# lucidrains/flash-cosine-sim-attention

Measured on AMD Instinct MI355X. Metric: attention TFLOP/s fwd+bwd (B=4,H=8,N=4096,D=64 bf16) + max-|delta| vs PyTorch ref, higher is better.
Workload: dtype bf16

## Files before the change

flash_cosine_sim_attention_amd/_lib.py:

```python
from __future__ import annotations

import ctypes as C
import os
import subprocess
import sys

_HERE = os.path.dirname(os.path.abspath(__file__))
LIB_PATH = os.environ.get("FCSA_LIB") or os.path.join(_HERE, "libfcsa_hip.so")
CSRC = os.path.join(_HERE, "csrc")

FCSA_F32, FCSA_F16, FCSA_BF16 = 0, 1, 2
_HEADER_CANDIDATES = (os.path.join(_HERE, "include", "fcsa.h"), os.path.join(os.path.dirname(_HERE), "include", "fcsa.h"))
HEADER = next((h for h in _HEADER_CANDIDATES if os.path.isfile(h)), _HEADER_CANDIDATES[0])



_SCALARS = {"int32_t": C.c_int32, "int64_t": C.c_int64, "uint64_t": C.c_uint64, "float": C.c_float, "size_t": C.c_size_t,
            "char": C.c_char, "int": C.c_int}


def _parse_header(path):
    import re
    text = re.sub(r"/\*.*?\*/", "", open(path).read(), flags=re.S)
    macros = {m.group(1): int(m.group(2)) for m in re.finditer(r"#define\s+(FCSA_\w+)\s+(-?\d+)\s*$", text, flags=re.M)}
    structs = {}
    for m in re.finditer(r"typedef\s+struct\s+(\w+)\s*\{(.*?)\}\s*(\w+)\s*;", text, flags=re.S):
        fields = []
        for decl in m.group(2).split(";"):
            decl = " ".join(decl.split())
            if not decl:
                continue
            head, _, names = decl.rpartition(" ")
            while "," in head:
                head, _, more = head.rpartition(" ")
                names = more + " " + names
            base = head.replace("const", "").strip()
            for nm in names.replace(",", " ").split():
                stars = base.count("*") + nm.count("*")
                nm = nm.strip("*")
                tname = base.replace("*", "").strip()
                arr = re.match(r"(\w+)\[(\d+)\]$", nm)
                if stars:
                    ct = C.c_void_p
                elif tname in structs:
                    ct = structs[tname][1]
                else:
                    ct = _SCALARS[tname]
                if arr:
                    nm, ct = arr.group(1), ct * int(arr.group(2))
                fields.append((nm, ct))
        cls = type(m.group(3), (C.Structure,), {"_fields_": fields})
        structs[m.group(3)] = (fields, cls)
    return {k: v[1] for k, v in structs.items()}, macros


_STRUCTS, _MACROS = _parse_header(HEADER)
ABI_VERSION = _MACROS["FCSA_ABI_VERSION"]
Tensor = _STRUCTS["fcsa_tensor"]
Problem = _STRUCTS["fcsa_problem"]
NormState = _STRUCTS["fcsa_norm_state"]
ForwardArgs = _STRUCTS["fcsa_forward_args"]
BackwardArgs = _STRUCTS["fcsa_backward_args"]
KernelStat = _STRUCTS["fcsa_kernel_stat"]
Varlen = _STRUCTS["fcsa_varlen"]
KvCache = _STRUCTS["fcsa_kvcache"]
Window = _STRUCTS["fcsa_window"]
KvCacheQuant = _STRUCTS["fcsa_kvcache_quant"]
FCSA_CACHE_E4M3 = _MACROS["FCSA_CACHE_E4M3"]
LseOut = _STRUCTS["fcsa_lse_out"]
MergeArgs = _STRUCTS["fcsa_merge_args"]
MERGE_MAX_STATES = _MACROS["FCSA_MERGE_MAX_STATES"]
MergeBackwardArgs = _STRUCTS["fcsa_merge_backward_args"]
KvCacheStep = _STRUCTS["fcsa_kvcache_step"]
STEP_CHUNK_ROWS = _MACROS["FCSA_STEP_CHUNK_ROWS"]
TreeMask = _STRUCTS["fcsa_tree_mask"]
Alibi = _STRUCTS["fcsa_alibi"]


EXPORTS = ("fcsa_forward", "fcsa_backward", "fcsa_backward_workspace_bytes", "fcsa_forward_workspace_bytes", "fcsa_forward_needs_qn",
           "fcsa_l2norm", "fcsa_debug", "fcsa_debug_forward_form", "fcsa_debug_kv_group_form", "fcsa_last_error", "fcsa_profile_enable", "fcsa_profile_collect",
           "fcsa_forward_varlen", "fcsa_backward_varlen", "fcsa_backward_varlen_workspace_bytes", "fcsa_forward_kvcache",
           "fcsa_forward_kvcache_workspace_bytes", "fcsa_forward_window", "fcsa_backward_window", "fcsa_backward_window_workspace_bytes",
           "fcsa_forward_kvcache_window", "fcsa_forward_kvcache_window_workspace_bytes", "fcsa_forward_kvcache_quant",
           "fcsa_forward_kvcache_quant_workspace_bytes", "fcsa_forward_kvcache_varlen", "fcsa_forward_kvcache_varlen_workspace_bytes",
           "fcsa_forward_kvcache_lse", "fcsa_merge_states", "fcsa_forward_kvcache_prefill",
           "fcsa_attention_lse", "fcsa_backward_state", "fcsa_merge_states_backward",
           "fcsa_forward_kvcache_step", "fcsa_forward_kvcache_step_workspace_bytes",
           "fcsa_forward_kvcache_tree", "fcsa_kvcache_compact", "fcsa_forward_kvcache_alibi")

_lib = None


def build(verbose: bool = False) -> str:
    cmd = ["make", "-C", CSRC, "-j", str(min(8, os.cpu_count() or 1)), "PYTHON=" + sys.executable]
    res = subprocess.run(cmd, capture_output=True, text=True)
    if verbose or res.returncode != 0:
        print(res.stdout)
        print(res.stderr)
    if res.returncode != 0:
        raise RuntimeError("building libfcsa_hip.so failed (see output above)")
    return LIB_PATH


def load():
    global _lib
    if _lib is not None:
        return _lib
    if not os.path.exists(LIB_PATH):
        raise ImportError(
            f"{LIB_PATH} is missing: the HIP extension has not been built. Run `make -C {CSRC}` "
            "(or `python -c 'import __graft_entry__ as g; g.build()'` at the repo root). "
            "There is no non-HIP fallback for GPU tensors.")
    lib = C.CDLL(LIB_PATH)
    lib.fcsa_forward.argtypes = [C.POINTER(ForwardArgs)]
    lib.fcsa_forward.restype = C.c_int
    lib.fcsa_backward.argtypes = [C.POINTER(BackwardArgs)]
    lib.fcsa_backward.restype = C.c_int
    lib.fcsa_backward_workspace_bytes.argtypes = [C.POINTER(Problem)]
    lib.fcsa_backward_workspace_bytes.restype = C.c_size_t
    lib.fcsa_forward_workspace_bytes.argtypes = [C.POINTER(Problem)]
    lib.fcsa_forward_workspace_bytes.restype = C.c_size_t
    lib.fcsa_forward_needs_qn.argtypes = [C.POINTER(Problem), C.c_int32]
    lib.fcsa_forward_needs_qn.restype = C.c_int
    lib.fcsa_l2norm.argtypes = [C.c_int32, C.c_int32, C.c_int32, C.c_int32, C.c_int32, C.c_int32,
                                C.POINTER(Tensor), C.c_void_p, C.c_void_p, C.c_void_p]
    lib.fcsa_l2norm.restype = C.c_int
    lib.fcsa_debug.argtypes = [C.c_char_p, C.c_size_t]
    lib.fcsa_debug.restype = C.c_int
    lib.fcsa_debug_forward_form.argtypes = [C.c_int32]
    lib.fcsa_debug_forward_form.restype = C.c_int
    lib.fcsa_debug_kv_group_form.argtypes = [C.c_int32]
    lib.fcsa_debug_kv_group_form.restype = C.c_int
    lib.fcsa_profile_enable.argtypes = [C.c_int32]
    lib.fcsa_profile_enable.restype = C.c_int
    lib.fcsa_profile_collect.argtypes = [C.POINTER(KernelStat), C.c_int32]
    lib.fcsa_profile_collect.restype = C.c_int
    lib.fcsa_forward_varlen.argtypes = [C.POINTER(ForwardArgs), C.POINTER(Varlen)]
    lib.fcsa_forward_varlen.restype = C.c_int
    lib.fcsa_backward_varlen.argtypes = [C.POINTER(BackwardArgs), C.POINTER(Varlen)]
    lib.fcsa_backward_varlen.restype = C.c_int
    lib.fcsa_backward_varlen_workspace_bytes.argtypes = [C.POINTER(Problem), C.POINTER(Varlen)]
    lib.fcsa_backward_varlen_workspace_bytes.restype = C.c_size_t
    lib.fcsa_forward_kvcache.argtypes = [C.POINTER(ForwardArgs), C.POINTER(KvCache)]
    lib.fcsa_forward_kvcache.restype = C.c_int
    lib.fcsa_forward_kvcache_workspace_bytes.argtypes = [C.POINTER(Problem), C.POINTER(KvCache)]
    lib.fcsa_forward_kvcache_workspace_bytes.restype = C.c_size_t
    if hasattr(lib, "fcsa_forward_window"):
        lib.fcsa_forward_window.argtypes = [C.POINTER(ForwardArgs), C.POINTER(Varlen), C.POINTER(Window)]
        lib.fcsa_forward_window.restype = C.c_int
        lib.fcsa_backward_window.argtypes = [C.POINTER(BackwardArgs), C.POINTER(Varlen), C.POINTER(Window)]
        lib.fcsa_backward_window.restype = C.c_int
        lib.fcsa_backward_window_workspace_bytes.argtypes = [C.POINTER(Problem), C.POINTER(Varlen), C.POINTER(Window)]
        lib.fcsa_backward_window_workspace_bytes.restype = C.c_size_t
        lib.fcsa_forward_kvcache_window.argtypes = [C.POINTER(ForwardArgs), C.POINTER(KvCache), C.POINTER(Window)]
        lib.fcsa_forward_kvcache_window.restype = C.c_int
        lib.fcsa_forward_kvcache_window_workspace_bytes.argtypes = [C.POINTER(Problem), C.POINTER(KvCache), C.POINTER(Window)]
        lib.fcsa_forward_kvcache_window_workspace_bytes.restype = C.c_size_t
    if hasattr(lib, "fcsa_forward_kvcache_quant"):
        lib.fcsa_forward_kvcache_quant.argtypes = [C.POINTER(ForwardArgs), C.POINTER(KvCache), C.POINTER(KvCacheQuant), C.POINTER(Window)]
        lib.fcsa_forward_kvcache_quant.restype = C.c_int
        lib.fcsa_forward_kvcache_quant_workspace_bytes.argtypes = [C.POINTER(Problem), C.POINTER(KvCache), C.POINTER(KvCacheQuant),
                                                                   C.POINTER(Window)]
        lib.fcsa_forward_kvcache_quant_workspace_bytes.restype = C.c_size_t
    if hasattr(lib, "fcsa_forward_kvcache_varlen"):
        lib.fcsa_forward_kvcache_varlen.argtypes = [C.POINTER(ForwardArgs), C.POINTER(KvCache), C.POINTER(Varlen), C.POINTER(KvCacheQuant),
                                                    C.POINTER(Window)]
        lib.fcsa_forward_kvcache_varlen.restype = C.c_int
        lib.fcsa_forward_kvcache_varlen_workspace_bytes.argtypes = [C.POINTER(Problem), C.POINTER(KvCache), C.POINTER(Varlen),
                                                                    C.POINTER(KvCacheQuant), C.POINTER(Window)]
        lib.fcsa_forward_kvcache_varlen_workspace_bytes.restype = C.c_size_t
    if hasattr(lib, "fcsa_forward_kvcache_lse"):
        lib.fcsa_forward_kvcache_lse.argtypes = [C.POINTER(ForwardArgs), C.POINTER(KvCache), C.POINTER(Varlen), C.POINTER(KvCacheQuant),
                                                 C.POINTER(Window), C.POINTER(LseOut)]
        lib.fcsa_forward_kvcache_lse.restype = C.c_int
        lib.fcsa_merge_states.argtypes = [C.POINTER(MergeArgs)]
        lib.fcsa_merge_states.restype = C.c_int
    if hasattr(lib, "fcsa_forward_kvcache_prefill"):
        lib.fcsa_forward_kvcache_prefill.argtypes = [C.POINTER(ForwardArgs), C.POINTER(KvCache), C.POINTER(Varlen), C.POINTER(LseOut)]
        lib.fcsa_forward_kvcache_prefill.restype = C.c_int
    if hasattr(lib, "fcsa_attention_lse"):
        lib.fcsa_attention_lse.argtypes = [C.POINTER(Problem), C.c_void_p, C.POINTER(Varlen), C.POINTER(Window), C.POINTER(LseOut), C.c_void_p]
        lib.fcsa_attention_lse.restype = C.c_int
        lib.fcsa_backward_state.argtypes = [C.POINTER(BackwardArgs), C.POINTER(Varlen), C.POINTER(Window), C.c_void_p]
        lib.fcsa_backward_state.restype = C.c_int
        lib.fcsa_merge_states_backward.argtypes = [C.POINTER(MergeBackwardArgs)]
        lib.fcsa_merge_states_backward.restype = C.c_int
    if hasattr(lib, "fcsa_forward_kvcache_step"):
        lib.fcsa_forward_kvcache_step.argtypes = [C.POINTER(ForwardArgs), C.POINTER(KvCache), C.POINTER(Varlen), C.POINTER(KvCacheQuant),
                                                  C.POINTER(Window), C.POINTER(KvCacheStep), C.POINTER(LseOut)]
        lib.fcsa_forward_kvcache_step.restype = C.c_int
        lib.fcsa_forward_kvcache_step_workspace_bytes.argtypes = [C.POINTER(Problem), C.POINTER(KvCache), C.POINTER(Varlen),
                                                                  C.POINTER(KvCacheQuant), C.POINTER(Window), C.POINTER(KvCacheStep)]
        lib.fcsa_forward_kvcache_step_workspace_bytes.restype = C.c_size_t
    if hasattr(lib, "fcsa_forward_kvcache_alibi"):
        lib.fcsa_forward_kvcache_alibi.argtypes = [C.POINTER(ForwardArgs), C.POINTER(KvCache), C.POINTER(Varlen), C.POINTER(KvCacheQuant),
                                                   C.POINTER(Window), C.POINTER(KvCacheStep), C.POINTER(Alibi), C.POINTER(LseOut)]
        lib.fcsa_forward_kvcache_alibi.restype = C.c_int
    if hasattr(lib, "fcsa_forward_kvcache_tree"):
        lib.fcsa_forward_kvcache_tree.argtypes = [C.POINTER(ForwardArgs), C.POINTER(KvCache), C.POINTER(Varlen), C.POINTER(KvCacheQuant),
                                                  C.POINTER(TreeMask), C.POINTER(LseOut)]
        lib.fcsa_forward_kvcache_tree.restype = C.c_int
        lib.fcsa_kvcache_compact.argtypes = [C.POINTER(KvCache), C.c_int32, C.c_int32, C.c_int32, C.c_int32, C.c_void_p, C.c_int64, C.c_int32,
                                             C.c_void_p, C.c_void_p]
        lib.fcsa_kvcache_compact.restype = C.c_int
    lib.fcsa_last_error.argtypes = []
    lib.fcsa_last_error.restype = C.c_char_p
    ver = lib.fcsa_debug(None, 0)
    if ver != ABI_VERSION:
        raise ImportError(f"libfcsa_hip.so ABI version {ver} != expected {ABI_VERSION}; rebuild it")
    _lib = lib
    return lib


def check(rc: int, what: str):
    if rc != 0:
        msg = load().fcsa_last_error().decode("utf-8", "replace")
        raise RuntimeError(f"{what} failed (status {rc}): {msg}")


def forward_form(form: int) -> int:
    return int(load().fcsa_debug_forward_form(int(form)))


def kv_group_form(form: int) -> int:
    return int(load().fcsa_debug_kv_group_form(int(form)))


def source_sha256() -> str:
    import hashlib
    h = hashlib.sha256()
    names = [f for f in sorted(os.listdir(CSRC)) if f.endswith((".hip", ".cuh", ".h", ".cpp")) or f == "Makefile"]
    names += ["dev/" + f for f in sorted(os.listdir(os.path.join(CSRC, "dev")))]
    for name, path in [(n, os.path.join(CSRC, n)) for n in names] + [(os.path.basename(HEADER), HEADER)]:
        h.update(name.encode() + b"\0")
        h.update(open(path, "rb").read())
    return h.hexdigest()


def profile_enable(on: bool):
    check(load().fcsa_profile_enable(1 if on else 0), "fcsa_profile_enable")


def profile_collect():
    arr = (KernelStat * 16)()
    n = load().fcsa_profile_collect(arr, 16)
    if n < 0:
        raise RuntimeError("fcsa_profile_collect failed")
    return [dict(name=arr[i].name.decode(), calls=arr[i].calls, total_ms=arr[i].total_ms, min_ms=arr[i].min_ms,
                 max_ms=arr[i].max_ms) for i in range(min(n, 16))]



def dtype_code(torch_dtype) -> int:
    import torch
    return {torch.float32: FCSA_F32, torch.float16: FCSA_F16, torch.bfloat16: FCSA_BF16}[torch_dtype]


def tensor4(t) -> "Tensor":
    assert t.dim() == 4 and t.stride(3) == 1
    return Tensor(t.data_ptr(), t.stride(0), t.stride(1), t.stride(2))


def problem(torch_dtype, dims, causal=False, bias_batch=False, l2norm_qk=True, groups=1, scale=8.0) -> "Problem":
    B, H, Hk, N, M, D = dims
    return Problem(dtype_code(torch_dtype), B, H, Hk, N, M, D, int(bool(causal)), int(bool(bias_batch)),
                   int(bool(l2norm_qk)), int(groups if l2norm_qk else 1), float(scale))


def forward_needs_qn(prob: "Problem", need_backward: bool) -> bool:
    return bool(load().fcsa_forward_needs_qn(C.byref(prob), 1 if need_backward else 0))
```

flash_cosine_sim_attention_amd/csrc/fcsa_bwd.hip:

```cpp
#include <type_traits>

#include "fcsa_common.cuh"
#include "fcsa_kernels.h"

namespace fcsa {
constexpr int kDqSub8 = 4;
constexpr bool kDqSplitFirstStage = true;
constexpr int kDkvBmq8 = 128;
constexpr int kDkvBmqWide = 64;
constexpr bool kDkvRing = true;
FCSA_TRACE_SITE(dq)
FCSA_TRACE_SITE(dkv)

template <typename T, int D, int MODE, bool BIAS, bool TWO, bool WIN = false>
FCSA_DEV void dq_tile(const char* kt, const char* vt, const FragAddr<T, D>& fa,
                      const u32x4 (&qf)[TileGeom<D, Traits<T>::ES>::KS], const u32x4 (&dof)[TileGeom<D, Traits<T>::ES>::KS],
                      f32x16 (&dq)[TileGeom<D, Traits<T>::ES>::DB], float lc, float delta, const BwdParams& p, uint64_t word,
                      uint32_t ncm, int i, int j0, int diff, const char* bias_row, int m_lim, int dlo = 0) {
  typedef TileGeom<D, Traits<T>::ES> G;
  typedef Traits<T> TR;
  constexpr bool MASKED = MODE == 1, KEYM = MODE == 2;
#pragma unroll
  for (int jb = 0; jb < 2; ++jb) {
    uint32_t w = 0xffffffffu;
// ... 1155 lines not shown
        reinterpret_cast<float*>(buf + 2 * TILE_B + BMQ * 4)[tid] = row_ok ? -dl_r : 0.f;
      }
    }
  };

  if constexpr (!DMA) {
    if (t0 < QT) load_tile(t0, smem);
  }

  u32x4 kf[G::KS], vf[G::KS];
#pragma unroll
  for (int kk = 0; kk < G::KS; ++kk) {
    kf[kk] = p.q_scaled ? rk_[kk] : scale_frag<T>(rk_[kk], p.c1);
    if constexpr (!LEAN) vf[kk] = rv_[kk];
  }
  float rinv[RowEpilogue<T, D>::NP];
  if constexpr (SEP) {
#pragma unroll
    for (int e = 0; e < RowEpilogue<T, D>::NP; ++e) rinv[e] = rinv_n[e];
  }
  const bool key_ok = j < p.M && rmask != 0;
  const uint32_t kmask = key_ok ? 0xffffffffu : 0u;
  const uint32_t ncm = causal ? 0u : 0xffffffffu;

  f32x16 dk[G::DB], dv[G::DB];
#pragma unroll
  for (int db = 0; db < G::DB; ++db)
#pragma unroll
    for (int r = 0; r < 16; ++r) { dk[db][r] = 0.f; dv[db][r] = 0.f; }

  if (t0 < QT) store_tile(smem);
  if constexpr (RING) {
    if ((SWEEP ? t0 < QT && (t0 + 1 < QT || p.kv_group > 1) : t0 + 1 < QT) && tid < BMQ) {
      char* buf1 = smem + BUF_B;
      reinterpret_cast<float*>(buf1 + 2 * TILE_B)[tid] = row_ok2 ? (p.invl_log2 ? lc_r2 : __builtin_amdgcn_logf(lc_r2)) - p.c2 : -INFINITY;
      reinterpret_cast<float*>(buf1 + 2 * TILE_B + BMQ * 4)[tid] = row_ok2 ? -dl_r2 : 0.f;
    }
  }
  if constexpr (LEAN) dma_wait();
  __syncthreads();
  __builtin_amdgcn_s_waitcnt(0x0F70);

  int t_m = QT;
  if (!BIAS && p.mask == nullptr && n0 + BNK <= p.M) {
    t_m = t0;
    if (causal) t_m = min(QT, max(t0, (nw + 31 - diff - hq + BMQ - 1) / BMQ));
  }
  int t_e = QT;
  if constexpr (WIN) win_unmasked_query_tiles(t0, QT, n0 + BNK <= p.M, nw, hq, BMS, BMQ, diff, dlo, t_m, t_e);
  const bool head_skip0 = SWEEP && causal && t_m > t0 && t0 * BMQ + hq + BMS - 1 + diff < nw;

  tr.loop_begin();
  DkvPipe<T, D, BMS> pipe;
  int pipe_tile = -1;
  int ring = 0;
  int tpar = 0;
  int gi = 0;
  auto run = [&](auto masked_tag, int t_begin, int t_end) {
    constexpr int MODE = decltype(masked_tag)::value;
    constexpr bool MASKED = MODE != 0;
    for (int t = t_begin; t < t_end; ++t) {
      const int i0 = t * BMQ;
      const int par = RING ? ring : SWEEP ? tpar : (t - t0) & 1;
      const int par_nxt = RING ? (ring == 2 ? 0 : ring + 1) : (par ^ 1);
      const int par_ld = RING ? (ring == 0 ? 2 : ring - 1) : (par ^ 1);
      const int t_ld = RING ? t + 2 : t + 1;
      const char* cur = smem + par * BUF_B;
      char* nxt = smem + par_ld * BUF_B;
      bool more = t_ld < QT;
      FCSA_STAMP(ts, 0);
      const float* lcs = reinterpret_cast<const float*>(cur + 2 * TILE_B);
      const float* dls = lcs + BMQ;
      if constexpr (SWEEP) {
        more = cursor_next(t0);
        if (more) load_rows(lt * BMQ);
      } else if constexpr (DMA) {
        if (more) {
          advance(t_ld);
          load_rows(t_ld * BMQ);
        }
      }
      if constexpr (DMA) {
        const uint32_t lds_nxt = lds0 + par_ld * BUF_B;
        FCSA_STAMP(ts, 1);
        if (more) {
          dq_.issue(stq, lds_nxt, wave);
          ddo_.issue(stdo, lds_nxt + TILE_B, wave);
        }
      } else {
        if (more) load_tile(t + 1, nxt);
        FCSA_STAMP(ts, 1);
      }
      {
      bool skip = false;
      if constexpr (MASKED) skip = causal && (i0 + hq + BMS - 1 + diff < nw);
      if constexpr (MASKED && WIN) skip = skip || (i0 + hq > nw + 31 - dlo);
      if constexpr (PIPE) {
        if constexpr (RING) {
          if (!skip) {
            const bool has_next = t + 1 < QT || (SWEEP && gi + 1 < p.kv_group && !head_skip0);
            if constexpr (QSPLIT)
              dkv_tile_pipe<T, D, BMS, tile_mode<MODE>(), true, true, WIN>(cur + hoff, cur + TILE_B + hoff, lcs + hq, dls + hq, fa, kf, vf, dk, dv, kmask, ncm, j, i0 + hq, diff, ts,
                                                          pipe, pipe_tile != t, has_next ? smem + par_nxt * BUF_B : cur, wave >= 4, hoff, hq, dlo);
            else
            dkv_tile_pipe<T, D, BMQ, tile_mode<MODE>(), true, false, WIN>(cur, cur + TILE_B, lcs, dls, fa, kf, vf, dk, dv, kmask, ncm, j, i0, diff, ts, pipe, pipe_tile != t,
                                                  has_next ? smem + par_nxt * BUF_B : cur, NW == 8 && wave >= 4, 0, 0, dlo);
            pipe_tile = has_next ? (t + 1 < QT ? t + 1 : t0) : -1;
          }
          ring = par_nxt;
        } else {
          if (!skip) dkv_tile_pipe<T, D, BMQ, tile_mode<MODE>(), false, false, WIN>(cur, cur + TILE_B, lcs, dls, fa, kf, vf, dk, dv, kmask, ncm, j, i0, diff, ts, pipe, true, nullptr,
                                                    NW == 8 && wave >= 4, 0, 0, dlo);
        }
      } else if constexpr (LEAN) {
        if (!skip) dkv_tile<T, D, BMQ, tile_mode<MODE>(), false, true, WIN>(cur, cur + TILE_B, lcs, dls, fa, kf, vf, dk, dv, p, kmask, ncm, j, i0, diff, nullptr, ts,
                                                            bb, bscr, nullptr, false, -1, lane, smem + LDS::VOWN, wave * 32, NW == 8 && wave >= 4, dlo);
      } else {
        const int next_i0 = more ? i0 + hq + BMQ : -1;
        if (!skip) {
          dkv_tile<T, D, BMS, tile_mode<MODE>(), BIAS, false, WIN>(cur + hoff, cur + TILE_B + hoff, lcs + hq, dls + hq, fa, kf, vf, dk, dv, p, kmask, ncm, j, i0 + hq, diff, bias_col, ts, bb, bscr,
                                            bias_blk, bvec, next_i0, lane, nullptr, 0, false, dlo);
        } else if constexpr (BIAS) {
          if (bvec && more) bb.request(bias_blk, min(next_i0 + (lane & 31), p.N - 1), (int64_t)p.M * TR::ES, fa.hi);
        }
      }
      }
      FCSA_STAMP(ts, 8);
      if (more) store_tile(nxt);
      if constexpr (SWEEP) tpar ^= 1;
      FCSA_STAMP(ts, 9);
      FCSA_BAR_BEGIN(tr);
      __syncthreads();
      FCSA_BAR_END(tr);
      FCSA_STAMP(ts, 10);
      if constexpr (!MASKED) ts.close(10);
    }
  };
  tr.mark(pass, 1);
  tpar = 0;
  for (gi = 0; gi < (SWEEP ? p.kv_group : 1); ++gi) {
    if constexpr (WIN) {
      int sb = t0, se = t_m, ub = t_m, ue = t_e;
#pragma nounroll
      for (int seg = 0; seg < 2; ++seg) {
        run(std::integral_constant<int, 1>{}, sb, se);
        run(std::integral_constant<int, 0>{}, ub, ue);
        sb = t_e; se = QT; ub = QT; ue = QT;
      }
    } else {
    run(std::integral_constant<int, KM ? 2 : 1>{}, t0, t_m);
    tr.mark(pass, 2);
    run(std::integral_constant<int, 0>{}, t_m, QT);
    }
  }
  tr.mark(pass, 3);
  tr.loop_end();

  if constexpr (QSPLIT) {
    LDS::HO::run(smem, rwave, half, lane, [&](int n) { return acc_x4(n & 4 ? dv : dk, n / 8 * 4 + n % 4); },
                 [&](int n, const f32x4& v) { add_x4(n & 4 ? dv : dk, n / 8 * 4 + n % 4, v); });
  }
  {
    typedef RowEpilogue<T, D> EP;
    char* scr = LDS::scratch(smem, rwave);
    char* xs = LDS::xarea(smem, rwave);
    const int rows_valid = half == 0 ? p.M - nw : 0;
    const bool fused = p.rk != nullptr;
    const int le = opaque(lane);
    const float kmul = p.q_scaled ? p.scale / p.c1 : p.scale;
    if constexpr (!SEP) {
#pragma unroll
      for (int e = 0; e < EP::NP; ++e) rinv[e] = 1.f;
      if (fused && rows_valid > 0) EP::load_inv(rinv, p.rk + (rk_bh * p.M + nw) * p.G, p.G, p.lgm, le, rows_valid);
    }
    if (rows_valid > 0) EP::put(scr, dk, kmul, le, (LDS::X && fused) ? kf : nullptr, xs, LDS::XPITCH);
    have_pre = false;
    if constexpr (SEP) {
      if (pass + 1 < npass) {
        request_ahead(pass + 1);
        have_pre = true;
      }
    }
    if (rows_valid > 0) {
      const int64_t split_off = p.dkv_splits > 1 ? (int64_t)blockIdx.y * p.dkv_split_stride : 0;
      const int ho = SWEEP ? hk : h;
      char* dk0 = p.dk.p + (int64_t)b * p.dk.sb + (int64_t)ho * p.dk.sh + (int64_t)nw * p.dk.sn + split_off;
      char* dv0 = p.dv.p + (int64_t)b * p.dv.sb + (int64_t)ho * p.dv.sh + (int64_t)nw * p.dv.sn + split_off;
      const char* x0 = fused ? p.k.p + (int64_t)b * p.k.sb + (int64_t)hk * p.k.sh + (int64_t)nw * p.k.sn : nullptr;
      EP::template finish<LDS::X>(scr, xs, LDS::XPITCH, le, dk0, p.dk.sn, rows_valid, fused ? false : p.dk_f32 != 0, x0, p.k.sn, 1.f, rinv, p.lgm,
                                  p.norm_eps);
      EP::put(scr, dv, 1.f, le, nullptr, xs, LDS::XPITCH);
      EP::template finish<false>(scr, xs, LDS::XPITCH, le, dv0, p.dv.sn, rows_valid, p.dv_f32 != 0, nullptr, 0, 1.f, rinv, 0, 1.f);
    }
    if constexpr (!SEP) {
      if (pass + 1 < npass) __syncthreads();
    }
  }
  tr.mark(pass, 4);
  }
  tr.finish(ts, wave, (wave & 2) == 0, trace_row8(wave));
}

template <typename T, int D, int NW, int BMQ, bool BIAS, bool LEAN, bool KM, bool RING = false, bool QSPLIT = false, bool SWEEP = false>
__global__ void __launch_bounds__(NW * 64, ((D * Traits<T>::ES <= kDkv2WBytes || LEAN) ? 2 : 1)) bwd_dkv_kernel(const BwdParams p_) {
  bwd_dkv_body<T, D, NW, BMQ, BIAS, LEAN, KM, RING, QSPLIT, SWEEP, false>(p_);
}
template <typename T, int D, int NW, int BMQ, bool LEAN, bool RING, bool QSPLIT>
__global__ void __launch_bounds__(NW * 64, ((D * Traits<T>::ES <= kDkv2WBytes || LEAN) ? 2 : 1)) bwd_dkv_win_kernel(const BwdWinParams p_) {
  bwd_dkv_body<T, D, NW, BMQ, false, LEAN, false, RING, QSPLIT, false, true>(p_);
}

template <typename T, int D, bool BIAS, int NW, bool TWO, bool KSPLIT = false>
static hipError_t launch_dq_nw(const BwdWinParams& p, hipStream_t s) {
  constexpr int SUB = KSPLIT ? 2 : NW == 8 ? (Traits<T>::ES == 2 ? kDqSub8 : 2) : 1;
  typedef DqLds<T, D, NW, SUB, TWO, KSPLIT> LDS;
  const dim3 grid((unsigned)((int64_t)p.B * p.H * tile_pairs(tile_count(p.N, 32 * LDS::RWAVES), p.causal)), (unsigned)(p.dq_splits > 1 ? p.dq_splits : 1));
  constexpr bool GENERAL_ONLY = TWO && D * Traits<T>::ES >= 256;
  if (p.window) {
    if constexpr (!BIAS && !(TWO && D * Traits<T>::ES > kDq2WBytes)) {
      if (!p.causal || p.dq_splits > 1 || p.mask != nullptr) return hipErrorInvalidValue;
      return launch_with_lds<bwd_dq_win_kernel<T, D, NW, SUB, TWO, KSPLIT>>(grid, dim3(NW * 64), LDS::TOTAL, s, p);
    }
    return hipErrorInvalidValue;
  }
  const BwdParams& bp = p;
  if constexpr (!GENERAL_ONLY) {
    if (!p.causal) return launch_with_lds<bwd_dq_kernel<T, D, NW, BIAS, SUB, TWO, true, KSPLIT>>(grid, dim3(NW * 64), LDS::TOTAL, s, bp);
  }
  return launch_with_lds<bwd_dq_kernel<T, D, NW, BIAS, SUB, TWO, false, KSPLIT>>(grid, dim3(NW * 64), LDS::TOTAL, s, bp);
}

template <typename T, int D, bool BIAS>
static hipError_t launch_dq_form(DqForm f, const BwdWinParams& p, hipStream_t s) {
  constexpr int ES = Traits<T>::ES;
  constexpr bool NARROW = D * ES <= kDq2WBytes;
  switch (f) {
    case DqForm::Waves4:
      return launch_dq_nw<T, D, BIAS, 4, NARROW>(p, s);
    case DqForm::Waves4Two:
      if constexpr (NARROW || (dq_can_two_waves(ES, D) && !BIAS)) return launch_dq_nw<T, D, BIAS, 4, true>(p, s);
      break;
    case DqForm::Waves8:
      if constexpr (NARROW) return launch_dq_nw<T, D, BIAS, 8, true>(p, s);
      break;
    case DqForm::KSplit8:
      if constexpr (bwd_ksplit(ES, D, false) && (NARROW || (dq_can_two_waves(ES, D) && !BIAS))) return launch_dq_nw<T, D, BIAS, 8, true, true>(p, s);
      break;
  }
  return hipErrorInvalidValue;
}

template <typename T, int D, bool BIAS, int NW, bool LEAN = false, bool QSPLIT = false, bool SWEEP = false>
static hipError_t launch_dkv_nw(const BwdWinParams& p, hipStream_t s) {
  constexpr bool DMA_FORM = Traits<T>::ES == 2 && !BIAS;
  constexpr int LEAN_BMQ = D * Traits<T>::ES < 256 ? 64 : 32;
  constexpr int BMQ = LEAN ? LEAN_BMQ : (D * Traits<T>::ES >= 192) ? (DMA_FORM ? kDkvBmqWide : 32) : (NW == 8 ? kDkvBmq8 : 64);
  constexpr bool RING = kDkvRing && DMA_FORM && !LEAN && (BMQ * TileGeom<D, Traits<T>::ES>::ROWB) % 1024 == 0 &&
                        DkvLds<T, D, NW, BMQ, BIAS, false, true, false>::FITS;
  typedef DkvLds<T, D, NW, BMQ, BIAS, LEAN, RING, QSPLIT> LDS;
  const dim3 grid((unsigned)(p.B * (SWEEP ? p.H / p.kv_group : p.H) * tile_pairs(tile_count(p.M, 32 * LDS::RWAVES), p.causal)),
                  (unsigned)(p.dkv_splits > 1 ? p.dkv_splits : 1));
  if (p.window) {
    if constexpr (!BIAS && !SWEEP) {
      if (!p.causal || p.dkv_splits > 1 || p.mask != nullptr) return hipErrorInvalidValue;
      return launch_with_lds<bwd_dkv_win_kernel<T, D, NW, BMQ, LEAN, RING, QSPLIT>>(grid, dim3(NW * 64), LDS::TOTAL, s, p);
    }
    return hipErrorInvalidValue;
  }
  const BwdParams& bp = p;
  return p.causal ? launch_with_lds<bwd_dkv_kernel<T, D, NW, BMQ, BIAS, LEAN, false, RING, QSPLIT, SWEEP>>(grid, dim3(NW * 64), LDS::TOTAL, s, bp)
                  : launch_with_lds<bwd_dkv_kernel<T, D, NW, BMQ, BIAS, LEAN, true, RING, QSPLIT, SWEEP>>(grid, dim3(NW * 64), LDS::TOTAL, s, bp);
}

static std::atomic<int> g_kv_group_mode{1};
int kv_group_mode(int set) {
  if (set < 0) return g_kv_group_mode.load(std::memory_order_relaxed);
  return g_kv_group_mode.exchange(set > 2 ? 2 : set, std::memory_order_relaxed);
}

template <typename T, int D, bool BIAS>
static hipError_t launch_dkv_form(DkvForm f, const BwdWinParams& p, hipStream_t s) {
  constexpr int ES = Traits<T>::ES;
  constexpr bool NARROW = D * ES <= kDkv2WBytes;
  switch (f) {
    case DkvForm::Waves4:
      return launch_dkv_nw<T, D, BIAS, 4>(p, s);
    case DkvForm::Waves8:
      if constexpr (NARROW) return launch_dkv_nw<T, D, BIAS, 8>(p, s);
      break;
    case DkvForm::Lean8:
      if constexpr (ES == 2 && !BIAS && !NARROW && D * ES <= 256) return launch_dkv_nw<T, D, BIAS, 8, true>(p, s);
      break;
    case DkvForm::QSplit8:
      if constexpr (NARROW && bwd_ksplit(ES, D, false)) return launch_dkv_nw<T, D, BIAS, 8, false, true>(p, s);
      break;
    case DkvForm::Sweep:
      if constexpr (dkv_has_sweep(ES, D, BIAS)) return launch_dkv_nw<T, D, BIAS, 8, !NARROW, false, true>(p, s);
      break;
  }
  return hipErrorInvalidValue;
}

static BwdProblem bwd_problem(int dtype, int D, const BwdWinParams& p, int splits) {
  return {dtype == 0 ? 4 : 2, D, (int64_t)p.B * p.H, p.N, p.M, p.causal != 0, p.bias != nullptr, splits, p.kv_sweep != 0,
          p.seq.cu_q != nullptr || p.window != 0, p.window != 0};
}

hipError_t launch_backward_dbias(int dtype, int D, const BwdParams& p, hipStream_t s) {
  if (p.B * p.H == 0 || p.N == 0 || p.M == 0 || p.d_bias == nullptr || p.bias == nullptr) return hipSuccess;
  return dispatch_dtype_d(dtype, D, [&](auto td) { return launch_dbias_t<typename decltype(td)::T, decltype(td)::D>(p, s); });
}

hipError_t launch_backward_dq(int dtype, int D, const BwdWinParams& p, hipStream_t s) {
  if (p.B * p.H == 0 || p.N == 0) return hipSuccess;
  const DqForm f = choose_dq(bwd_problem(dtype, D, p, p.dq_splits), cu_count());
  return dispatch_dtype_d(dtype, D, [&](auto td) {
    using T = typename decltype(td)::T;
    constexpr int DD = decltype(td)::D;
    return p.bias != nullptr ? launch_dq_form<T, DD, true>(f, p, s) : launch_dq_form<T, DD, false>(f, p, s);
  });
}

hipError_t launch_backward_dkv(int dtype, int D, const BwdWinParams& p, hipStream_t s) {
  if (p.B * p.H == 0 || p.M == 0) return hipSuccess;
  const DkvForm f = choose_dkv(bwd_problem(dtype, D, p, p.dkv_splits), cu_count());
  return dispatch_dtype_d(dtype, D, [&](auto td) {
    using T = typename decltype(td)::T;
    constexpr int DD = decltype(td)::D;
    return p.bias != nullptr ? launch_dkv_form<T, DD, true>(f, p, s) : launch_dkv_form<T, DD, false>(f, p, s);
  });
}

}
```

flash_cosine_sim_attention_amd/csrc/fcsa_capi.hip:

```cpp
#include "../../include/fcsa.h"
#include "fcsa_kernels.h"

#include <algorithm>
#include <cstdarg>
#include <cstdio>
#include <cmath>
#include <cstring>
#include <atomic>
#include <mutex>
#include <string>
#include <vector>

namespace {

thread_local std::string g_err;
constexpr float kLog2e = 1.4426950408889634f;

int fail(int code, const char* fmt, ...) {
  char buf[512];
  va_list ap;
  va_start(ap, fmt);
  vsnprintf(buf, sizeof(buf), fmt, ap);
  va_end(ap);
  g_err = buf;
  return code;
}

int elem_size(int dtype) { return dtype == FCSA_F32 ? 4 : 2; }

size_t align_up(size_t x, size_t a) { return (x + a - 1) / a * a; }

bool dim_ok(int d) { return d == 16 || d == 32 || d == 64 || d == 96 || d == 128; }

int check_problem(const fcsa_problem& p) {
  if (p.dtype != FCSA_F16 && p.dtype != FCSA_BF16 && p.dtype != FCSA_F32)
    return fail(FCSA_ERR_UNSUPPORTED, "unsupported dtype %d (expected f32=0, f16=1, bf16=2)", p.dtype);
  if (!dim_ok(p.dim_head))
    return fail(FCSA_ERR_UNSUPPORTED, "dim_head %d not in {16, 32, 64, 96, 128}", p.dim_head);
  if (p.batch < 0 || p.heads < 0 || p.q_len < 0 || p.k_len < 0)
    return fail(FCSA_ERR_INVALID_ARG, "negative size (B=%d H=%d N=%d M=%d)", p.batch, p.heads, p.q_len, p.k_len);
  if (p.kv_heads < 1 ? p.heads != 0 || p.kv_heads != 0 : p.heads % p.kv_heads != 0)
    return fail(FCSA_ERR_INVALID_ARG, "kv_heads must divide heads (%d), got %d", p.heads, p.kv_heads);
  if (p.l2norm_qk) {
    if (p.groups < 1 || p.dim_head % p.groups != 0)
      return fail(FCSA_ERR_INVALID_ARG, "groups (%d) must divide dim_head (%d)", p.groups, p.dim_head);
    if (p.dtype == FCSA_F16 && fabsf(p.scale) * kLog2e > 60000.f)
      return fail(FCSA_ERR_UNSUPPORTED, "float16: scale %g puts scale * log2(e) * q^ outside the type", (double)p.scale);
  } else if (p.groups != 1) {
    return fail(FCSA_ERR_INVALID_ARG, "groups must be 1 when l2norm_qk is 0");
  }
  if (!(p.scale == p.scale) || std::isinf(p.scale)) return fail(FCSA_ERR_INVALID_ARG, "scale is NaN or infinite");
  return FCSA_OK;
}

int check_tensor(const char* name, const fcsa_tensor& t, int es, bool required) {
  if (t.ptr == nullptr) return required ? fail(FCSA_ERR_INVALID_ARG, "%s: null pointer", name) : FCSA_OK;
  if ((reinterpret_cast<uintptr_t>(t.ptr) & 15) != 0) return fail(FCSA_ERR_INVALID_ARG, "%s: base not 16-byte aligned", name);
  const int64_t m = 16 / es;
  if (t.stride0 % m || t.stride1 % m || t.stride2 % m)
    return fail(FCSA_ERR_INVALID_ARG, "%s: strides (%lld, %lld, %lld) must keep rows 16-byte aligned", name,
                (long long)t.stride0, (long long)t.stride1, (long long)t.stride2);
  if (t.stride2 < 0 || t.stride2 * es > (int64_t)(0x3fffffff / 256))
    return fail(FCSA_ERR_UNSUPPORTED, "%s: row stride %lld elements is negative or above 4 MiB", name, (long long)t.stride2);
  return FCSA_OK;
}

fcsa::View view(const fcsa_tensor& t, int es, bool zero_head_stride = false) {
  fcsa::View v;
  v.p = static_cast<char*>(t.ptr);
  v.sb = t.stride0 * es;
  v.sh = zero_head_stride ? 0 : t.stride1 * es;
  v.sn = t.stride2 * es;
  return v;
}

fcsa::View contiguous_view(void* p, int64_t heads, int64_t len, int64_t d, int es, bool zero_head_stride = false) {
  fcsa::View v;
  v.p = static_cast<char*>(p);
  v.sb = heads * len * d * es;
  v.sh = zero_head_stride ? 0 : len * d * es;
  v.sn = d * es;
  return v;
}

constexpr float kStaticTop = 65.f, kStaticBottom = 85.f;
constexpr float kStaticBoundBias = 40.f;
bool dynamic_shift(const fcsa_problem& p, bool has_bias) {
  if (!p.l2norm_qk) return false;
  const float bound = fabsf(p.scale) * (float)p.groups;
  if (p.dtype == FCSA_F16) return has_bias || bound > 11.f;
  return 2.f * bound > kStaticTop + kStaticBottom || (has_bias && bound > kStaticBoundBias);
}

float exponent_shift(const fcsa_problem& p, bool has_bias) {
  if (!p.l2norm_qk) return p.scale;
  if (dynamic_shift(p, has_bias)) return 0.f;
  const float bound = fabsf(p.scale) * (float)p.groups;
  if (p.dtype == FCSA_F16) return bound - 10.f;
  const float lo = bound - kStaticTop, hi = kStaticBottom - bound;
  return p.scale < lo ? lo : (p.scale > hi ? hi : p.scale);
}

float rowsum_eps(const fcsa_problem& p, bool has_bias) {
  if (dynamic_shift(p, has_bias)) return 1e-30f;
  float e = 1e-10f * expf(p.scale - exponent_shift(p, has_bias));
  if (!(e > 1e-37f)) e = 1e-37f;
  if (e > 1e30f) e = 1e30f;
  return e;
}

int log2_blocks_per_group(const fcsa_problem& p) {
  const int dg = p.dim_head / (p.groups > 0 ? p.groups : 1);
  if (dg % 8 != 0) return -1;
  int m = dg / 8, lg = 0;
  while ((1 << lg) < m) ++lg;
  if (p.groups <= 1) return lg;
  return (1 << lg) == m ? lg : -1;
}
bool fusable_groups(const fcsa_problem& p) { return log2_blocks_per_group(p) >= 0; }

struct BwdPlan {
  bool fuse_norm;
  bool kv_sweep;
  int dq_splits;
  int dkv_splits;
  bool dq_slab, dk_slab, dv_slab;
};
struct BwdCall { bool bias, dq_flat, dkv_flat; };

BwdPlan bwd_plan(const fcsa_problem& p, const BwdCall* call, bool varlen = false) {
  BwdPlan b;
  const int cus = fcsa::cu_count();
  const bool grouped = p.kv_heads != p.heads;
  const bool sweep = !varlen && p.kv_heads > 1 && grouped && (p.l2norm_qk == 0 || fusable_groups(p)) &&
                     fcsa::dkv_sweep(elem_size(p.dtype), p.dim_head, (int64_t)p.batch * p.kv_heads, p.k_len, p.causal != 0, fcsa::kv_group_mode(-1), cus);
  b.kv_sweep = sweep && call != nullptr && !call->bias;
  b.fuse_norm = p.l2norm_qk != 0 && fusable_groups(p);
  const bool norm_slab = p.l2norm_qk != 0 && !b.fuse_norm;
  b.dq_splits = varlen || (call != nullptr && !(call->dq_flat && !(p.causal && call->bias))) ? 1 : fcsa::backward_dq_splits(p, cus);
  b.dkv_splits = varlen || sweep || (call != nullptr && !((call->dkv_flat || grouped) && !call->bias)) ? 1 : fcsa::backward_dkv_splits(p, cus);
  b.dq_slab = b.dq_splits > 1 || norm_slab;
  b.dk_slab = !b.kv_sweep && (b.dkv_splits > 1 || grouped || norm_slab);
  b.dv_slab = !b.kv_sweep && (b.dkv_splits > 1 || grouped);
  return b;
}

struct BwdLayout { size_t delta, dq_slab, dk_slab, dv_slab, total; };
BwdLayout bwd_layout(const fcsa_problem& p, bool varlen = false) {
  const BwdPlan b = bwd_plan(p, nullptr, varlen);
  const size_t qn = (size_t)p.batch * p.heads * p.q_len;
  const size_t kn = (size_t)p.batch * p.heads * p.k_len;
  BwdLayout L;
  size_t off = 0;
  L.delta = off;   off = align_up(off + qn * 4, 256);
  L.dq_slab = off; off = align_up(off + (b.dq_slab ? qn * p.dim_head * 4 * (size_t)b.dq_splits : 0), 256);
  L.dk_slab = off; off = align_up(off + (b.dk_slab ? kn * p.dim_head * 4 * (size_t)b.dkv_splits : 0), 256);
  L.dv_slab = off; off = align_up(off + (b.dv_slab ? kn * p.dim_head * 4 * (size_t)b.dkv_splits : 0), 256);
  L.total = off;
  return L;
}

int launch_check(hipError_t e, const char* what) {
  if (e != hipSuccess) return fail(FCSA_ERR_LAUNCH, "%s: %s", what, hipGetErrorString(e));
  return FCSA_OK;
}

struct TimedLaunch { const char* name; hipEvent_t start, stop; };
std::mutex g_prof_mu;
std::atomic<bool> g_prof_on{false};
std::vector<TimedLaunch> g_prof;

template <typename F> int timed(const char* name, const char* what, hipStream_t s, F&& launch) {
  if (!g_prof_on.load(std::memory_order_relaxed)) return launch_check(launch(), what);
  TimedLaunch t{name, nullptr, nullptr};
  if (hipEventCreate(&t.start) != hipSuccess || hipEventCreate(&t.stop) != hipSuccess)
    return fail(FCSA_ERR_LAUNCH, "%s: hipEventCreate failed", what);
  (void)hipEventRecord(t.start, s);
  const hipError_t e = launch();
  (void)hipEventRecord(t.stop, s);
  { std::lock_guard<std::mutex> g(g_prof_mu); g_prof.push_back(t); }
  return launch_check(e, what);
}

int check_varlen(const fcsa_problem& p, const fcsa_varlen* v, bool mask, bool bias) {
  if (v == nullptr) return fail(FCSA_ERR_INVALID_ARG, "varlen: null sequence table");
  if (mask || bias) return fail(FCSA_ERR_INVALID_ARG, "varlen: mask and attn_bias are not supported with packed sequences");
  if (v->total_q < 0 || v->total_k < 0 || v->total_q > INT32_MAX || v->total_k > INT32_MAX)
    return fail(FCSA_ERR_INVALID_ARG, "varlen: total_q / total_k (%lld, %lld) outside [0, 2^31)", (long long)v->total_q, (long long)v->total_k);
  if (p.batch > 0 && (v->cu_seqlens_q == nullptr || v->cu_seqlens_k == nullptr))
    return fail(FCSA_ERR_INVALID_ARG, "varlen: null cu_seqlens");
  if ((int64_t)p.heads * (v->total_q > v->total_k ? v->total_q : v->total_k) > INT32_MAX)
    return fail(FCSA_ERR_UNSUPPORTED, "varlen: heads x packed rows above 2^31");
  return FCSA_OK;
}
fcsa_problem packed_problem(const fcsa_problem& p, const fcsa_varlen& v) {
  fcsa_problem d = p;
  d.batch = 1;
  d.q_len = (int32_t)v.total_q;
  d.k_len = (int32_t)v.total_k;
  return d;
}
struct VarlenCall { const fcsa_varlen* t; int batch, max_q, max_k; };
fcsa::SeqTable seq_table(const VarlenCall* v) {
  if (v == nullptr) return fcsa::SeqTable{nullptr, nullptr, 0, 0};
  return fcsa::SeqTable{v->t->cu_seqlens_q, v->t->cu_seqlens_k, (int)v->t->total_q, (int)v->t->total_k};
}
fcsa_tensor packed(fcsa_tensor t) {
  t.stride0 = 0;
  return t;
}

struct WindowCall { int lo, hi; };
int check_window(const fcsa_window* w, bool mask, bool bias) {
  if (w == nullptr) return fail(FCSA_ERR_INVALID_ARG, "window: null window");
  if (w->left < -1 || w->right < -1) return fail(FCSA_ERR_INVALID_ARG, "window: left / right (%d, %d) must be >= 0, or -1 for unbounded", w->left, w->right);
  if (mask || bias) return fail(FCSA_ERR_INVALID_ARG, "window: mask and attn_bias are not supported with a sliding window");
  return FCSA_OK;
}

int forward_impl(const fcsa_forward_args* a, const VarlenCall* vl, const WindowCall* win = nullptr);
int backward_impl(const fcsa_backward_args* a, const VarlenCall* vl, const WindowCall* win = nullptr, const float* dlse = nullptr);

}

extern "C" {

const char* fcsa_last_error(void) { return g_err.c_str(); }

int fcsa_profile_enable(int32_t enable) {
  g_prof_on.store(enable != 0, std::memory_order_relaxed);
  return FCSA_OK;
}

int fcsa_profile_collect(fcsa_kernel_stat* stats, int32_t capacity) {
  std::vector<TimedLaunch> rec;
  { std::lock_guard<std::mutex> g(g_prof_mu); rec.swap(g_prof); }
  std::vector<fcsa_kernel_stat> agg;
  for (TimedLaunch& t : rec) {
    float ms = 0.f;
    const bool ok = hipEventSynchronize(t.stop) == hipSuccess && hipEventElapsedTime(&ms, t.start, t.stop) == hipSuccess;
    (void)hipEventDestroy(t.start);
    (void)hipEventDestroy(t.stop);
    if (!ok) continue;
    fcsa_kernel_stat* st = nullptr;
    for (auto& a : agg) if (strcmp(a.name, t.name) == 0) st = &a;
    if (st == nullptr) {
      fcsa_kernel_stat n;
      memset(&n, 0, sizeof(n));
      strncpy(n.name, t.name, sizeof(n.name) - 1);
      n.min_ms = ms; n.max_ms = ms;
      agg.push_back(n);
      st = &agg.back();
    }
    st->calls += 1;
    st->total_ms += ms;
    if (ms < st->min_ms) st->min_ms = ms;
    if (ms > st->max_ms) st->max_ms = ms;
  }
  if (stats != nullptr)
    for (int i = 0; i < (int)agg.size() && i < capacity; ++i) stats[i] = agg[i];
  return (int)agg.size();
}

int fcsa_debug(char* buf, size_t buf_bytes) {
  if (buf != nullptr && buf_bytes > 0) {
    snprintf(buf, buf_bytes,
             "libfcsa_hip abi=%d arch=gfx950 dtypes=f32,f16,bf16 dim_head=16,32,64,96,128 "
             "kernels=l2norm,l2norm_pair,fwd(32 rows/wave; lean two-wave form at D=96/128),fwd2(64 rows/wave),fwd3(D=128: 64 rows/wave, 1 wave/SIMD),fwd_ksplit(128 rows, wave halves split the keys),fwd_split+combine,"
             "fwd_dyn(per-row shift),bwd_dq(+split-key; key-split form on 8 waves),bwd_dkv(+lean; query-split form on 8 waves; grouped-query K/V head sweep),bwd_dbias,finalize,kv_append+decode+decode_combine(kv cache),"
             "window(fwd_win,bwd_dq_win,bwd_dkv_win,decode_win: sliding-window forms),"
             "kv_append_fp8+decode_fp8+decode_combine_fp8(e4m3fn kv cache, f16/bf16 queries),"
             "kv_append_ragged+decode_ragged+decode_combine_ragged(+_fp8: packed queries with per-sequence counts against the kv cache),"
             "decode_tree(+_fp8: a per-row bit set over the step's tokens, tree attention for speculative decoding)+kv_compact(the accepted path to the front of its slots) kv_heads=divisors of heads",
             FCSA_ABI_VERSION);
  }
  return FCSA_ABI_VERSION;
}

int fcsa_debug_forward_form(int32_t form) { return fcsa::forward_wide128_mode(form); }

int fcsa_debug_kv_group_form(int32_t form) { return fcsa::kv_group_mode(form); }

int fcsa_l2norm(int32_t dtype, int32_t batch, int32_t heads, int32_t len, int32_t dim_head, int32_t groups,
                const fcsa_tensor* x, void* xn, float* inv_norm, void* stream) {
  if (dtype != FCSA_F16 && dtype != FCSA_BF16 && dtype != FCSA_F32) return fail(FCSA_ERR_UNSUPPORTED, "fcsa_l2norm: dtype %d not supported", dtype);
  if (batch < 0 || heads < 0 || len < 0) return fail(FCSA_ERR_INVALID_ARG, "fcsa_l2norm: negative size (B=%d H=%d L=%d)", batch, heads, len);
  if (batch == 0 || heads == 0 || len == 0) return FCSA_OK;
  if (x == nullptr || xn == nullptr) return fail(FCSA_ERR_INVALID_ARG, "fcsa_l2norm: null argument");
  if (dim_head <= 0 || dim_head % 8 != 0) return fail(FCSA_ERR_UNSUPPORTED, "fcsa_l2norm: dim_head %d must be a multiple of 8", dim_head);
  if (dim_head > 512) return fail(FCSA_ERR_UNSUPPORTED, "fcsa_l2norm: dim_head %d > 512", dim_head);
  if (groups < 1 || dim_head % groups != 0) return fail(FCSA_ERR_INVALID_ARG, "fcsa_l2norm: groups (%d) must divide dim_head (%d)", groups, dim_head);
  const int es = elem_size(dtype);
  if (int rc = check_tensor("x", *x, es, true)) return rc;
  fcsa::NormParams np;
  np.x = view(*x, es);
  np.xn = static_cast<char*>(xn);
  np.inv_norm = inv_norm;
  np.B = batch; np.H = heads; np.L = len; np.D = dim_head; np.G = groups;
  np.eps = 1e-12f;
  np.out_scale = 1.f;
  hipStream_t s = static_cast<hipStream_t>(stream);
  return timed("l2norm", "l2norm", s, [&] { return fcsa::launch_l2norm(dtype, np, s); });
}

static int forward_splits(const fcsa_problem& p) {
  if (p.batch <= 0 || p.heads <= 0 || p.q_len <= 0 || p.dim_head <= 0) return 1;
  return fcsa::forward_splits(p, dynamic_shift(p, false), fcsa::cu_count());
}
static size_t forward_ws_bytes(const fcsa_problem& p, int splits) {
  if (splits <= 1) return 0;
  const size_t rows = (size_t)splits * p.batch * p.heads * p.q_len;
  return align_up(rows * p.dim_head * 4, 256) + align_up(rows * 4, 256);
}

size_t fcsa_forward_workspace_bytes(const fcsa_problem* p) { return p == nullptr ? 0 : forward_ws_bytes(*p, forward_splits(*p)); }

static int zero_rows(const char* name, const fcsa_tensor& t, int es, int B, int H, int L, int D, hipStream_t s) {
  if (B <= 0 || H <= 0 || L <= 0) return FCSA_OK;
  if (int rc = check_tensor(name, t, es, true)) return rc;
  for (int b = 0; b < B; ++b)
    for (int h = 0; h < H; ++h) {
      char* base = static_cast<char*>(t.ptr) + ((int64_t)b * t.stride0 + (int64_t)h * t.stride1) * es;
      const hipError_t e = t.stride2 == D ? hipMemsetAsync(base, 0, (size_t)L * D * es, s)
                                          : hipMemset2DAsync(base, (size_t)t.stride2 * es, 0, (size_t)D * es, (size_t)L, s);
      if (e != hipSuccess) return fail(FCSA_ERR_LAUNCH, "%s: zero fill failed: %s", name, hipGetErrorString(e));
    }
  return FCSA_OK;
}

int fcsa_forward(const fcsa_forward_args* a) { return forward_impl(a, nullptr); }

static int forward_varlen(const fcsa_forward_args* a, const fcsa_varlen* seqs, const WindowCall* win) {
  if (a == nullptr) return fail(FCSA_ERR_INVALID_ARG, "null args");
  if (int rc = check_problem(a->p)) return rc;
  if (int rc = check_varlen(a->p, seqs, a->mask != nullptr, a->attn_bias != nullptr)) return rc;
  fcsa_forward_args pa = *a;
  pa.q = packed(pa.q); pa.k = packed(pa.k); pa.v = packed(pa.v); pa.o = packed(pa.o);
  pa.p = packed_problem(a->p, *seqs);
  const VarlenCall vl = {seqs, a->p.batch, a->p.q_len, a->p.k_len};
  return forward_impl(&pa, &vl, win);
}
int fcsa_forward_varlen(const fcsa_forward_args* a, const fcsa_varlen* seqs) { return forward_varlen(a, seqs, nullptr); }

int fcsa_forward_window(const fcsa_forward_args* a, const fcsa_varlen* seqs, const fcsa_window* w) {
  if (a == nullptr) return fail(FCSA_ERR_INVALID_ARG, "null args");
  if (int rc = check_problem(a->p)) return rc;
  if (int rc = check_window(w, a->mask != nullptr, a->attn_bias != nullptr)) return rc;
  WindowCall win;
  const fcsa::WinKind kind = fcsa::win_normalise(a->p.q_len, a->p.k_len, a->p.causal != 0, w->left, w->right, win.lo, win.hi);
  if (kind == fcsa::WinKind::Window) return seqs != nullptr ? forward_varlen(a, seqs, &win) : forward_impl(a, nullptr, &win);
  fcsa_forward_args na = *a;
  na.p.causal = kind == fcsa::WinKind::Causal ? 1 : 0;
  return seqs != nullptr ? fcsa_forward_varlen(&na, seqs) : fcsa_forward(&na);
}


}

namespace {

struct DecodeCall {
  const fcsa_forward_args* a;
  const fcsa_kvcache* kv;
  const fcsa_varlen* seqs;
  const fcsa_kvcache_quant* qz;
  const fcsa_window* w;
  const fcsa_lse_out* lse;
  const fcsa_kvcache_step* step = nullptr;
  const fcsa_tree_mask* tree = nullptr;
  const fcsa_alibi* alibi = nullptr;
};

struct DecodeWindow {
  int windowed, lo, hi, causal;
  int reach() const { return windowed ? lo : fcsa::kWinOpen; }
};
DecodeWindow decode_window(const fcsa_problem& p, const fcsa_kvcache& kv, bool ragged, const fcsa_window* w) {
  if (ragged) {
    const int lo = w == nullptr || w->left < 0 ? fcsa::kWinOpen : std::min(w->left, fcsa::kWinOpen);
    const int hi = p.causal ? 0 : (w == nullptr || w->right < 0 ? fcsa::kWinOpen : std::min(w->right, fcsa::kWinOpen));
    return {1, lo, hi, p.causal};
  }
  if (w == nullptr) return {0, 0, 0, p.causal};
  int lo, hi;
  const int max_k = std::min(std::max(p.k_len, 0), std::max(kv.capacity, 0));
  const fcsa::WinKind kind = fcsa::win_normalise(p.q_len, max_k, p.causal != 0, w->left, w->right, lo, hi);
  if (kind == fcsa::WinKind::Window) return {1, lo, hi, p.causal};
  return {0, 0, 0, kind == fcsa::WinKind::Causal ? 1 : 0};
}

struct DecodePlan { int row_tiles; int64_t slots; int splits; size_t ws_ml, total; };
DecodePlan decode_plan(const fcsa_problem& p, const fcsa_kvcache& kv, const fcsa_varlen* seqs, int win_lo, int64_t decode_rows = -1) {
  DecodePlan d;
  const int G = p.kv_heads > 0 ? p.heads / p.kv_heads : 0;
  const int max_k = fcsa::win_decode_keys(std::min(std::max(p.k_len, 0), std::max(kv.capacity, 0)), std::max(p.q_len, 0), win_lo);
  size_t rows;
  if (seqs != nullptr) {
    const int64_t total_q = std::max<int64_t>(seqs->total_q, 0);
    d.row_tiles = 0;
    d.slots = fcsa::ragged_slots(total_q, std::max(p.batch, 0), G);
    const int64_t split_slots = decode_rows < 0 ? d.slots : fcsa::ragged_slots(std::min(decode_rows, total_q), std::max(p.batch, 0), G);
    d.splits = fcsa::decode_splits(1, p.kv_heads, (int)std::min<int64_t>(split_slots, INT32_MAX), max_k, p.dim_head, fcsa::cu_count());
    rows = (size_t)total_q * std::max(p.heads, 0);
  } else {
    d.row_tiles = std::max(fcsa::decode_row_tiles(G * p.q_len), 1);
    d.slots = 0;
    d.splits = fcsa::decode_splits(p.batch, p.kv_heads, d.row_tiles, max_k, p.dim_head, fcsa::cu_count());
    rows = (size_t)std::max(p.batch, 0) * std::max(p.heads, 0) * std::max(p.q_len, 0);
  }
  d.ws_ml = align_up(rows * d.splits * std::max(p.dim_head, 0) * 4, 256);
  d.total = rows == 0 ? 0 : d.ws_ml + align_up(rows * d.splits * 8, 256);
  return d;
}
size_t decode_workspace_bytes(const fcsa_problem* p, const fcsa_kvcache* kv, const fcsa_varlen* seqs, const fcsa_window* w) {
  if (p == nullptr || kv == nullptr) return 0;
  return decode_plan(*p, *kv, seqs, decode_window(*p, *kv, seqs != nullptr, w).reach()).total;
}

int check_kvcache(const fcsa_forward_args* a, const fcsa_kvcache* kv, int cache_es = 0) {
  if (a == nullptr || kv == nullptr) return fail(FCSA_ERR_INVALID_ARG, "kvcache: null argument");
  const fcsa_problem& p = a->p;
  if (int rc = check_problem(p)) return rc;
  if (a->inv_l != nullptr || a->mask != nullptr || a->attn_bias != nullptr)
    return fail(FCSA_ERR_INVALID_ARG, "kvcache: inv_l, mask and attn_bias must be NULL (forward only, no mask or bias)");
  if (kv->capacity < 0 || kv->new_len < 0) return fail(FCSA_ERR_INVALID_ARG, "kvcache: negative capacity (%d) or new_len (%d)", kv->capacity, kv->new_len);
  if (kv->block_table != nullptr) {
    if (kv->page_size <= 0 || kv->page_size % 16 != 0) return fail(FCSA_ERR_INVALID_ARG, "kvcache: page_size %d must be a positive multiple of 16", kv->page_size);
    if (kv->capacity % kv->page_size != 0) return fail(FCSA_ERR_INVALID_ARG, "kvcache: capacity %d is not a whole number of pages of %d", kv->capacity, kv->page_size);
    if (kv->capacity > 0 && kv->num_blocks < 1) return fail(FCSA_ERR_INVALID_ARG, "kvcache: paged cache without blocks");
    if (kv->block_table_stride < kv->capacity / kv->page_size) return fail(FCSA_ERR_INVALID_ARG, "kvcache: block_table row stride %lld below %d entries", (long long)kv->block_table_stride, kv->capacity / kv->page_size);
  } else if (kv->page_size != 0) {
    return fail(FCSA_ERR_INVALID_ARG, "kvcache: page_size %d without a block_table", kv->page_size);
  }
  const int es = elem_size(p.dtype);
  const bool rows = p.batch > 0 && p.heads > 0 && p.q_len > 0;
  const bool cache = p.batch > 0 && kv->capacity > 0;
  const int ces = cache_es > 0 ? cache_es : es;
  if (rows) {
    if (int rc = check_tensor("q", a->q, es, true)) return rc;
    if (int rc = check_tensor("o", a->o, es, true)) return rc;
  }
  if (cache) {
    if (int rc = check_tensor("k_cache", kv->k_cache, ces, true)) return rc;
    if (int rc = check_tensor("v_cache", kv->v_cache, ces, true)) return rc;
  }
  if (cache && kv->new_len > 0) {
    if (int rc = check_tensor("k_new", kv->k_new, es, true)) return rc;
    if (int rc = check_tensor("v_new", kv->v_new, es, true)) return rc;
  }
  if (rows) {
    const DecodePlan d = decode_plan(p, *kv, nullptr, fcsa::kWinOpen);
    if ((int64_t)p.batch * p.kv_heads * d.row_tiles * d.splits > INT32_MAX) return fail(FCSA_ERR_UNSUPPORTED, "kvcache: grid above 2^31 workgroups");
  }
  return FCSA_OK;
}

int check_quant(const fcsa_forward_args* a, const fcsa_kvcache* kv, const fcsa_kvcache_quant* qz) {
  if (a == nullptr || kv == nullptr || qz == nullptr) return fail(FCSA_ERR_INVALID_ARG, "kvcache_quant: null argument");
  if (qz->cache_dtype != FCSA_CACHE_E4M3)
    return fail(FCSA_ERR_UNSUPPORTED, "kvcache_quant: cache type %d not supported (expected FCSA_CACHE_E4M3 = %d, OCP e4m3fn)", qz->cache_dtype, FCSA_CACHE_E4M3);
  if (a->p.dtype == FCSA_F32) return fail(FCSA_ERR_UNSUPPORTED, "kvcache_quant: float32 queries with an fp8 cache are not supported (f16 or bf16)");
  if (qz->k_scale == nullptr || qz->v_scale == nullptr) return fail(FCSA_ERR_INVALID_ARG, "kvcache_quant: null k_scale / v_scale");
  return check_kvcache(a, kv, 1);
}

int check_kvcache_varlen(const DecodeCall& c) {
  const fcsa_forward_args* a = c.a;
  const fcsa_kvcache* kv = c.kv;
  const fcsa_varlen* seqs = c.seqs;
  if (a == nullptr || kv == nullptr || seqs == nullptr) return fail(FCSA_ERR_INVALID_ARG, "kvcache_varlen: null argument");
  if (seqs->total_q < 0 || seqs->total_q > INT32_MAX) return fail(FCSA_ERR_INVALID_ARG, "kvcache_varlen: total_q (%lld) outside [0, 2^31)", (long long)seqs->total_q);
  if (a->p.batch > 0 && seqs->cu_seqlens_q == nullptr) return fail(FCSA_ERR_INVALID_ARG, "kvcache_varlen: null cu_seqlens_q");
  if (kv->new_len != 0 && kv->new_len != 1) return fail(FCSA_ERR_INVALID_ARG, "kvcache_varlen: new_len (%d) is a flag here: 0 (no append) or 1 (every query row brings its key and value)", kv->new_len);
  if (c.w != nullptr)
    if (int rc = check_window(c.w, false, false)) return rc;
  fcsa_forward_args pa = *a;
  fcsa_kvcache pk = *kv;
  pa.q = packed(pa.q); pa.o = packed(pa.o);
  pk.k_new = packed(pk.k_new); pk.v_new = packed(pk.v_new);
  pa.p.q_len = (int32_t)seqs->total_q;
  pa.p.batch = std::min(a->p.batch, 1);
  pk.new_len = kv->new_len != 0 && seqs->total_q > 0 ? 1 : 0;
  if (a->p.q_len < 0) return fail(FCSA_ERR_INVALID_ARG, "kvcache_varlen: negative max_seqlen_q (%d)", a->p.q_len);
  if ((int64_t)std::max(a->p.heads, 0) * seqs->total_q > INT32_MAX) return fail(FCSA_ERR_UNSUPPORTED, "kvcache_varlen: heads x packed rows above 2^31");
  return c.qz != nullptr ? check_quant(&pa, &pk, c.qz) : check_kvcache(&pa, &pk);
}

struct LaunchName { const char* name; const char* what; };
constexpr LaunchName kAppendName[2][2] = {{{"kv_append", "kv append"}, {"kv_append_fp8", "kv append (fp8)"}},
                                          {{"kv_append_ragged", "kv append (ragged)"}, {"kv_append_ragged_fp8", "kv append (ragged)"}}};
constexpr LaunchName kDecodeName[2][2] = {{{"decode", "decode"}, {"decode_fp8", "decode (fp8)"}},
                                          {{"decode_ragged", "decode (ragged)"}, {"decode_ragged_fp8", "decode (ragged)"}}};
constexpr LaunchName kCombineName[2][2][2] = {
    {{{"decode_combine", "decode combine"}, {"decode_combine_lse", "decode combine (lse)"}},
     {{"decode_combine_fp8", "decode combine (fp8)"}, {"decode_combine_lse_fp8", "decode combine (lse, fp8)"}}},
    {{{"decode_combine_ragged", "decode combine (ragged)"}, {"decode_combine_lse_ragged", "decode combine (lse, ragged)"}},
     {{"decode_combine_ragged_fp8", "decode combine (ragged)"}, {"decode_combine_lse_ragged_fp8", "decode combine (lse, ragged)"}}}};

fcsa::DecodeStepParams decode_params(const DecodeCall& c, const DecodeWindow& win, const DecodePlan& d) {
  const bool ragged = c.seqs != nullptr, fp8 = c.qz != nullptr;
  const fcsa_forward_args* a = c.a;
  const fcsa_kvcache* kv = c.kv;
  const fcsa_problem& p = a->p;
  const int es = elem_size(p.dtype), ces = fp8 ? 1 : es;
  auto rows_view = [&](const fcsa_tensor& t) { return view(ragged ? packed(t) : t, es); };
  fcsa::DecodeStepParams dp{};
  dp.q = rows_view(a->q);
  dp.o = rows_view(a->o);
  dp.kc = view(kv->k_cache, ces);
  dp.vc = view(kv->v_cache, ces);
  dp.kn = rows_view(kv->k_new);
  dp.vn = rows_view(kv->v_new);
  dp.seqlens = kv->cache_seqlens;
  dp.table = kv->block_table;
  dp.table_stride = kv->block_table_stride;
  dp.capacity = kv->capacity;
  dp.page = kv->block_table != nullptr ? kv->page_size : 0;
  dp.num_blocks = kv->num_blocks;
  dp.new_len = ragged ? 0 : kv->new_len;
  dp.B = p.batch; dp.H = p.heads; dp.Hk = p.kv_heads; dp.G = p.heads / p.kv_heads; dp.N = ragged ? 0 : p.q_len;
  dp.row_tiles = d.row_tiles; dp.splits = d.splits;
  dp.causal = win.causal; dp.l2norm = p.l2norm_qk; dp.groups = p.l2norm_qk ? p.groups : 1;
  dp.c1 = p.scale * kLog2e;
  dp.c2 = exponent_shift(p, false) * kLog2e;
  dp.l_eps = rowsum_eps(p, false);
  dp.dyn = dynamic_shift(p, false) ? 1 : 0;
  dp.ws_o = static_cast<float*>(a->workspace);
  dp.ws_ml = a->workspace != nullptr ? reinterpret_cast<float*>(static_cast<char*>(a->workspace) + d.ws_ml) : nullptr;
  dp.window = win.windowed; dp.win_lo = win.lo; dp.win_hi = win.hi;
  if (fp8) {
    dp.k_scale = c.qz->k_scale; dp.v_scale = c.qz->v_scale;
    dp.ks_b = c.qz->k_scale_stride0; dp.ks_h = c.qz->k_scale_stride1;
    dp.vs_b = c.qz->v_scale_stride0; dp.vs_h = c.qz->v_scale_stride1;
  }
  if (ragged) {
    dp.cu_q = c.seqs->cu_seqlens_q;
    dp.total_q = (int)c.seqs->total_q;
    dp.slots = (int)d.slots;
    dp.append = kv->new_len != 0 ? 1 : 0;
  }
  if (c.alibi != nullptr) {
    dp.c2 = 0.f;
    dp.l_eps = 1e-30f;
    dp.dyn = 1;
  }
  return dp;
}

fcsa::DecodeLseOut lse_view(const fcsa_lse_out& l, bool packed = false) { return {l.lse, packed ? 0 : l.stride0, l.stride1, l.stride2}; }

bool has_chunk_kernel(const fcsa_problem& p) { return p.dtype != FCSA_F32 && (p.dim_head == 64 || p.dim_head == 128); }

int check_workspace(const char* who, const fcsa_forward_args& a, const DecodePlan& d) {
  if (a.workspace == nullptr || a.workspace_bytes < d.total)
    return fail(FCSA_ERR_WORKSPACE, "%s: workspace too small: %zu < %zu bytes", who, a.workspace_bytes, d.total);
  if ((reinterpret_cast<uintptr_t>(a.workspace) & 255) != 0) return fail(FCSA_ERR_WORKSPACE, "%s: workspace not 256-byte aligned", who);
  return FCSA_OK;
}

int append_launch(const DecodeCall& c, fcsa::DecodeForm form, const fcsa::DecodeStepParams& dp, hipStream_t s) {
  if (c.kv->new_len <= 0 || c.kv->capacity <= 0) return FCSA_OK;
  const LaunchName& n = kAppendName[form.ragged][form.fp8];
  return timed(n.name, n.what, s, [&] { return fcsa::launch_kv_append(c.a->p.dtype, c.a->p.dim_head, form, dp, s); });
}

fcsa::DecodeAlibi alibi_view(const fcsa_alibi& al) { return {al.slopes, al.stride_b, al.stride_h}; }
constexpr LaunchName kAlibiDecodeName[2] = {{"alibi_decode", "decode (alibi)"}, {"alibi_decode_fp8", "decode (alibi, fp8)"}};
constexpr LaunchName kAlibiPrefillName[2] = {{"alibi_prefill", "prefill (alibi)"}, {"alibi_prefill_fp8", "prefill (alibi, fp8)"}};

int decode_launch(const LaunchName& plain, const DecodeCall& c, fcsa::DecodeForm form, const fcsa::DecodeStepParams& dp, hipStream_t s) {
  const fcsa_problem& p = c.a->p;
  if (c.alibi == nullptr) return timed(plain.name, plain.what, s, [&] { return fcsa::launch_decode(p.dtype, p.dim_head, form, dp, s); });
  const LaunchName& n = kAlibiDecodeName[form.fp8];
  const fcsa::DecodeAlibi al = alibi_view(*c.alibi);
  return timed(n.name, n.what, s, [&] { return fcsa::launch_decode_alibi(p.dtype, p.dim_head, form, dp, al, s); });
}

int chunk_launch(const LaunchName& plain, const DecodeCall& c, fcsa::DecodeForm form, fcsa::DecodeStepParams dp, int64_t slots, hipStream_t s) {
  dp.slots = (int)slots;
  dp.splits = 1;
  dp.ws_o = nullptr;
  dp.ws_ml = nullptr;
  const fcsa::DecodeLseOut lo = c.lse != nullptr ? lse_view(*c.lse, true) : fcsa::DecodeLseOut{};
  const fcsa::DecodeLseOut* lse = c.lse != nullptr ? &lo : nullptr;
// ... 684 lines not shown
```

flash_cosine_sim_attention_amd/csrc/fcsa_dispatch.h:

```cpp
#pragma once
#include <stdint.h>
#include <algorithm>
#include <cmath>

#include "../../include/fcsa.h"
#ifdef FCSA_VAR_SPLIT_ENV
#include "dev/fcsa_sweep_env.h"
namespace fcsa {
inline int sweep_env(const char* name) { return fcsa_dev::env_int(name); }
constexpr bool kSweepBuild = true;
}
#else
namespace fcsa {
constexpr int sweep_env(const char*) { return -1; }
constexpr bool kSweepBuild = false;
}
#endif

namespace fcsa {

constexpr int kDq2WBytes = 128;
constexpr int kDkv2WBytes = 128;

constexpr bool fwd_lean(int es, int D, bool bias) { return es == 2 && !bias && D * es > 128 && D * es <= 256; }
// ... 5 lines not shown

enum class FwdForm { Rows8, Lean8, KSplit8, Waves4, Fwd2, Fwd3 };
enum class DqForm { Waves4, Waves4Two, Waves8, KSplit8 };
enum class DkvForm { Waves4, Waves8, Lean8, QSplit8, Sweep };

constexpr int tile_count(int len, int tile) { return (len + tile - 1) / tile; }
constexpr int tile_pairs(int tiles, int causal) { return causal ? (tiles + 1) / 2 : tiles; }
constexpr int pair_passes(int tiles, int pair, int causal) { return (causal && (tiles - 1 - pair) != pair) ? 2 : 1; }
constexpr int pass_tile(int tiles, int pair, int pass, int causal, bool rows) {
  return causal ? (rows ? (pass == 0 ? tiles - 1 - pair : pair) : (pass == 0 ? pair : tiles - 1 - pair)) : pair;
}

constexpr void block_work(int id, int n_bh, int pairs, int& bh, int& pair) {
  if ((n_bh & 7) == 0) {
    const int xcd = id & 7, slot = id >> 3;
    bh = (slot / pairs) * 8 + xcd;
    pair = slot % pairs;
  } else {
    bh = id / pairs;
    pair = id % pairs;
  }
}

constexpr void key_split(int M, int split, int splits, int bn, int& lo, int& len) {
  const int tps = ((M + bn - 1) / bn + splits - 1) / splits;
  lo = split * tps * bn;
  len = std::max(std::min(lo + tps * bn, M) - lo, 0);
}
constexpr void key_split_causal(int N, int M, int m0, int bm, int split, int splits, int bn, int& lo, int& len) {
  const int vis = std::max(std::min(m0 + bm + M - N, M), 0);
  const int tps = std::max(((vis + bn - 1) / bn + splits - 1) / splits, 1);
  lo = std::min(M, split * tps * bn);
  len = std::max(std::min(lo + tps * bn, M) - lo, 0);
}
constexpr int key_tiles(int len, int m0, int bm, int diff, int causal, int bn) {
  int last_key = len - 1;
  if (causal) last_key = std::min(m0 + bm - 1 + diff, last_key);
  return last_key < 0 ? 0 : last_key / bn + 1;
}
constexpr void query_split(int tiles, int split, int splits, int& lo, int& hi) {
  const int tps = (tiles + splits - 1) / splits;
  lo = split * tps;
  hi = std::min(lo + tps, tiles);
}
constexpr int diagonal_tile(int n0, int diff, int bmq) { return std::max(n0 - diff, 0) / bmq; }
constexpr void query_split_causal(int tiles, int first, int split, int splits, int& lo, int& hi) {
  const int tps = std::max((tiles - first + splits - 1) / splits, 1);
  lo = std::min(first + split * tps, tiles);
  hi = std::min(lo + tps, tiles);
}

constexpr int kWinOpen = 1 << 28;
enum class WinKind { Full, Causal, Window };
constexpr WinKind win_normalise(int N, int M, bool causal, int left, int right, int& lo, int& hi) {
  hi = causal ? 0 : (right < 0 || right >= N - 1) ? kWinOpen : right;
  lo = (left < 0 || left >= M - 1) ? kWinOpen : left;
  return lo != kWinOpen ? WinKind::Window : hi == kWinOpen ? WinKind::Full : hi == 0 ? WinKind::Causal : WinKind::Window;
}
constexpr void win_key_window(int N, int M, int m0, int bm, int lo, int hi, int bn, int& k_lo, int& len) {
  const int d = M - N, r1 = std::min(m0 + bm, N) - 1;
  const int first = std::max(m0 + d - lo, 0), last = std::min(r1 + d + hi, M - 1);
  k_lo = 0;
  len = 0;
  if (r1 < m0 || last < first) return;
  k_lo = first / bn * bn;
  len = last + 1 - k_lo;
}
constexpr void win_unmasked_tiles(int len, int nt, int mw, int rows, int diff, int dlo, int bn, int& a, int& b) {
  const int hi_t = std::min(len / bn, std::max(0, mw + diff + 1) / bn);
  const int edge = mw + rows - 1 + dlo;
  a = std::min(edge <= 0 ? 0 : (edge + bn - 1) / bn, nt);
  b = std::max(a, std::min(hi_t, nt));
}
constexpr void win_query_tiles(int N, int M, int n0, int bnk, int lo, int hi, int bmq, int& t0, int& t1) {
  const int d = M - N, k1 = std::min(n0 + bnk, M) - 1;
  const int first = std::max(n0 - d - hi, 0), last = std::min(k1 - d + lo, N - 1);
  t0 = 0;
  t1 = 0;
  if (k1 < n0 || last < first) return;
  t0 = first / bmq;
  t1 = last / bmq + 1;
}
constexpr void win_unmasked_query_tiles(int t0, int t1, bool whole, int nw, int hq, int bms, int bmq, int diff, int dlo, int& a, int& b) {
  a = t1;
  b = t1;
  if (!whole) return;
  a = std::min(t1, std::max(t0, (nw + 31 - diff - hq + bmq - 1) / bmq));
  const int64_t x = (int64_t)nw - dlo - hq - bms + 1;
  b = std::min<int64_t>(t1, std::max<int64_t>(a, x < 0 ? 0 : x / bmq + 1));
}
constexpr void seq_span(int64_t lo, int64_t hi, int total, int max_len, int& start, int& len) {
  const int64_t st = std::min(std::max(lo, (int64_t)0), (int64_t)total);
  const int64_t en = std::min(std::max(hi, st), (int64_t)total);
  start = (int)st;
  len = (int)std::min(en - st, (int64_t)std::max(max_len, 0));
}
constexpr bool seq_pair_idle(int pair, int len, int tile, int causal) { return pair >= tile_pairs(tile_count(len, tile), causal); }

constexpr int kDecodeRows = 16;
constexpr int kDecodeBlock = 32;
constexpr int kDecodeMaxSplits = 128;
constexpr int kDecodeWavesPerCu = 8;
constexpr int decode_row_tiles(int groups_x_queries) { return (groups_x_queries + kDecodeRows - 1) / kDecodeRows; }
constexpr int decode_min_split_keys(int D) { return std::max(16384 / std::max(D, 1), kDecodeBlock); }
inline int decode_splits(int64_t batch, int kv_heads, int row_tiles, int max_k, int D, int cus) {
  const int64_t base = batch * (int64_t)kv_heads * row_tiles;
  if (base <= 0 || max_k <= 0) return 1;
  int64_t s = ((int64_t)cus * kDecodeWavesPerCu + base - 1) / base;
  s = std::min<int64_t>(s, std::max(1, max_k / decode_min_split_keys(D)));
  s = std::min<int64_t>(s, kDecodeMaxSplits);
  return (int)std::max<int64_t>(s, 1);
}
constexpr void decode_window(int len, int split, int splits, int& lo, int& n) {
  const int per = (std::max(len, 0) + splits - 1) / std::max(splits, 1);
  const int chunk = (per + kDecodeBlock - 1) / kDecodeBlock * kDecodeBlock;
  lo = std::min(split * chunk, std::max(len, 0));
  n = std::max(std::min(lo + chunk, len) - lo, 0);
}
constexpr int decode_len(bool has_table, int64_t cached, int new_len, int capacity) {
  const int64_t c = has_table ? std::min<int64_t>(std::max<int64_t>(cached, 0), capacity) : capacity;
  return (int)std::min<int64_t>(c + std::max(new_len, 0), capacity);
}
constexpr bool decode_groups_fast(int D, int groups, int unit) {
  if (groups < 1 || D % groups != 0) return false;
  const int gs = D / groups;
  if (groups == 1 || unit % gs == 0) return true;
  if (gs % unit != 0) return false;
  const int u = gs / unit;
  return (u & (u - 1)) == 0;
}

constexpr int win_decode_first(int len, int N, int lo) {
  return lo >= kWinOpen ? 0 : std::max(len - N - lo, 0) / kDecodeBlock * kDecodeBlock;
}
constexpr int win_decode_keys(int max_k, int N, int lo) {
  return lo >= kWinOpen ? max_k : (int)std::min<int64_t>(max_k, (int64_t)lo + N + kDecodeBlock - 1);
}

constexpr int64_t ragged_cu(int64_t raw, int64_t total) { return std::min(std::max(raw, (int64_t)0), total); }
constexpr int64_t ragged_base(int64_t cu_b, int b, int G) { return (int64_t)G * cu_b / kDecodeRows + b; }
constexpr int64_t ragged_slots(int64_t total_q, int64_t B, int G) { return (int64_t)G * total_q / kDecodeRows + B; }
constexpr int ragged_seq_of(const int32_t* cu, int B, int64_t total, int64_t tok) {
  int lo = 0, hi = B - 1;
  while (lo < hi) {
    const int mid = (lo + hi + 1) / 2;
    if (ragged_cu(cu[mid], total) <= tok) lo = mid; else hi = mid - 1;
  }
  return lo;
}
constexpr bool ragged_tile(const int32_t* cu, int B, int64_t total, int G, int64_t slot, int& b, int& rt, int& start, int& len) {
  int lo = 0, hi = B - 1;
  while (lo < hi) {
    const int mid = (lo + hi + 1) / 2;
    if (ragged_base(ragged_cu(cu[mid], total), mid, G) <= slot) lo = mid; else hi = mid - 1;
  }
  const int64_t st = ragged_cu(cu[lo], total), en = std::max(ragged_cu(cu[lo + 1], total), st);
  const int64_t t = slot - ragged_base(st, lo, G);
  b = lo;
  start = (int)st;
  len = (int)(en - st);
  rt = (int)t;
  return t >= 0 && t < ((int64_t)G * (en - st) + kDecodeRows - 1) / kDecodeRows;
}

constexpr int kPrefillRows = 128;
constexpr int kPrefillStage = 64;
constexpr int64_t prefill_base(int64_t cu_b, int b, int G, int rows) { return (int64_t)G * cu_b / rows + b; }
constexpr int64_t prefill_slots(int64_t total_q, int64_t B, int G, int rows) { return (int64_t)G * total_q / rows + B; }
constexpr bool prefill_tile(const int32_t* cu, int B, int64_t total, int G, int rows, int64_t slot, int& b, int& rt, int& start, int& len) {
  int lo = 0, hi = B - 1;
  while (lo < hi) {
    const int mid = (lo + hi + 1) / 2;
    if (prefill_base(ragged_cu(cu[mid], total), mid, G, rows) <= slot) lo = mid; else hi = mid - 1;
  }
  const int64_t st = ragged_cu(cu[lo], total), en = std::max(ragged_cu(cu[lo + 1], total), st);
  const int64_t t = slot - prefill_base(st, lo, G, rows);
  b = lo;
  start = (int)st;
  len = (int)(en - st);
  rt = (int)t;
  return t >= 0 && t < ((int64_t)G * (en - st) + rows - 1) / rows;
}
constexpr int prefill_kend(int L, int N, int G, int64_t first, int count, bool causal) {
  const int64_t last = std::min(first + count, (int64_t)G * N) - 1;
  if (last < first || L <= 0) return 0;
  if (!causal) return L;
  return (int)std::min<int64_t>(std::max<int64_t>((int64_t)L - N + last / G + 1, 0), L);
}
constexpr int prefill_kstart(int L, int N, int G, int64_t first, int lo) {
  if (lo >= kWinOpen) return 0;
  return (int)(std::max<int64_t>((int64_t)L - N + first / G - lo, 0) / kPrefillStage * kPrefillStage);
}
constexpr int prefill_win_kend(int L, int N, int G, int64_t first, int count, int hi) {
  if (hi >= kWinOpen || hi == 0) return prefill_kend(L, N, G, first, count, hi == 0);
  const int64_t last = std::min(first + count, (int64_t)G * N) - 1;
  if (last < first || L <= 0) return 0;
  return (int)std::min<int64_t>(std::max<int64_t>((int64_t)L - N + last / G + hi + 1, 0), L);
}
constexpr bool step_is_chunk(int G, int64_t N, int chunk_rows) { return (int64_t)G * N >= chunk_rows; }
constexpr int kStepChunkRows = 1024;

#if defined(__HIPCC__)
#define FCSA_HOST_DEVICE __host__ __device__
#else
#define FCSA_HOST_DEVICE
#endif
constexpr int kMergeMaxStates = 8;
FCSA_HOST_DEVICE inline float decode_row_lse(float M, float l) {
  if (!(M > -INFINITY) || !(l > 0.f)) return -INFINITY;
  return (float)(0.6931471805599453 * ((double)M + log2((double)l)));
}
FCSA_HOST_DEVICE inline float merge_row_weights(const float* lse, int S, float* w, float& lse_out) {
  float M = -INFINITY;
  for (int s = 0; s < S; ++s) M = lse[s] > M ? lse[s] : M;
  if (!(M > -INFINITY)) {
    for (int s = 0; s < S; ++s) w[s] = 0.f;
    lse_out = -INFINITY;
    return 0.f;
  }
  float W = 0.f;
  for (int s = 0; s < S; ++s) {
    w[s] = lse[s] > -INFINITY ? expf(lse[s] - M) : 0.f;
    W += w[s];
  }
  lse_out = M + logf(W);
  return W;
}

inline int64_t tile_workgroups(int64_t batch_heads, int len, int tile, bool causal) {
  return batch_heads * tile_pairs(tile_count(len, tile), causal);
}

inline int tile_waves(int64_t batch_heads, int len, bool causal, bool bits16, int tail, int cus) {
  const int64_t w256 = tile_workgroups(batch_heads, len, 256, causal);
  if (bits16 && tail != 0 && w256 > cus) {
    const int64_t rem = w256 % cus;
    if (tail == 2) return rem != 0 ? 4 : 8;
    return (rem != 0 && rem * 20 <= (int64_t)cus * 11) ? 4 : 8;
  }
  if (w256 >= cus * 7 / 8) return 8;
  if (bits16 && tile_workgroups(batch_heads, len, 128, causal) > cus) return 8;
  return 4;
}

inline bool fwd_ksplit_pays(int es, int D, int64_t workgroups, int cus) { return D * es > 128 || workgroups <= cus; }

struct FwdProblem {
  int es, D;
  int64_t batch_heads;
  int N, M;
  bool causal, bias, mask, dyn;
  int splits;
  int64_t q_row_bytes, k_row_bytes, v_row_bytes;
  int wide128_mode;
  bool varlen = false;
};

inline bool fwd3_applies(const FwdProblem& f, int cus) {
  if (f.D != 128 || f.es != 2 || f.bias || f.mask || f.dyn || f.splits > 1 || f.wide128_mode == 0) return false;
  if (tile_workgroups(f.batch_heads, f.N, 256, f.causal) < cus * 7 / 8) {
    if (tile_workgroups(f.batch_heads, f.N, 128, f.causal) <= cus || f.M < 2048) return false;
  }
  if ((int64_t)(f.M + 64 * 6) * f.k_row_bytes >= 0x7fffffffLL || (int64_t)(f.M + 64 * 6) * f.v_row_bytes >= 0x7fffffffLL) return false;
  return (int64_t)(f.N + 256) * f.q_row_bytes < 0x7fffffffLL;
}

inline bool fwd2_applies(const FwdProblem& f) {
  if (f.es != 2 || f.D != 32 || f.bias || f.dyn || f.splits > 1 || f.mask) return false;
  if (tile_workgroups(f.batch_heads, f.N, 256, f.causal) < 224) return false;
  return f.causal ? f.N >= 8192 : f.M >= 4096;
}

inline FwdForm choose_forward(const FwdProblem& f, int cus) {
  const int env = sweep_env("FCSA_FWD_FORM"), env_ks = sweep_env("FCSA_KSPLIT");
  const bool plain = !f.bias && !f.mask && !f.dyn && f.splits <= 1 && !f.varlen;
  if (f.varlen) {
  } else if (env > 0) {
    if (env == 5 && f.D == 128 && f.es == 2 && plain) return FwdForm::Fwd3;
    if (env == 4 && fwd2_compiled(f.es, f.D) && plain) return FwdForm::Fwd2;
  } else {
    if (fwd3_applies(f, cus)) return FwdForm::Fwd3;
    if (fwd2_applies(f)) return FwdForm::Fwd2;
  }
  const bool narrow = f.D * f.es <= 128, lean = fwd_lean(f.es, f.D, f.bias);
  const bool ksplit = fwd_ksplit(f.es, f.D, f.bias) &&
      (env_ks >= 0 ? env_ks != 0 : fwd_ksplit_pays(f.es, f.D, tile_workgroups(f.batch_heads, f.N, 128, f.causal) * std::max(f.splits, 1), cus));
  if (!f.dyn && f.splits > 1) return ksplit ? FwdForm::KSplit8 : FwdForm::Waves4;
  if (!f.dyn && fwd_ksplit(f.es, f.D, f.bias) && (narrow || lean) && env >= 1 && env <= 3)
    return env == 1 ? (narrow ? FwdForm::Rows8 : FwdForm::Lean8) : env == 2 ? FwdForm::KSplit8 : FwdForm::Waves4;
  if (narrow && tile_waves(f.batch_heads, f.N, f.causal, f.es == 2, 1, cus) == 8) return FwdForm::Rows8;
  if (!narrow && lean && tile_waves(f.batch_heads, f.N, f.causal, true, 0, cus) == 8) return FwdForm::Lean8;
  return ksplit ? FwdForm::KSplit8 : FwdForm::Waves4;
}

struct BwdProblem {
  int es, D;
  int64_t batch_heads;
  int N, M;
  bool causal, bias;
  int splits;
  bool kv_sweep;
  bool varlen = false;
  bool window = false;
};

inline DqForm choose_dq(const BwdProblem& b, int cus) {
  if (b.splits > 1 && !b.varlen) return DqForm::Waves4;
  const bool narrow = b.D * b.es <= kDq2WBytes, two = dq_can_two_waves(b.es, b.D) && !b.bias;
  if (b.window && !narrow) return DqForm::Waves4;
  if (const int env = sweep_env("FCSA_DQ_FORM"); bwd_ksplit(b.es, b.D, b.bias) && (narrow || two)) {
    if (env == 1) return narrow ? DqForm::Waves8 : DqForm::Waves4Two;
    if (env == 2 && (narrow || b.causal)) return DqForm::KSplit8;
    if (env == 3) return DqForm::Waves4;
  }
  const int64_t wgs128 = tile_workgroups(b.batch_heads, b.N, 128, b.causal);
  if (narrow) {
    if (tile_waves(b.batch_heads, b.N, b.causal, b.es == 2, 2, cus) == 8) return DqForm::Waves8;
    if (bwd_ksplit(b.es, b.D, false) && wgs128 <= cus) return DqForm::KSplit8;
  } else if (two) {
    if (wgs128 > cus) return DqForm::Waves4Two;
    if (bwd_ksplit(b.es, b.D, b.bias) && b.causal) return DqForm::KSplit8;
  }
  return DqForm::Waves4;
}

inline bool dkv_sweep(int es, int D, int64_t batch_kv_heads, int M, bool causal, int mode, int cus) {
  if (!dkv_has_sweep(es, D, false) || mode <= 0) return false;
  return mode >= 2 || tile_waves(batch_kv_heads, M, causal, true, 1, cus) == 8;
}

inline DkvForm choose_dkv(const BwdProblem& b, int cus) {
  if (b.kv_sweep && !b.varlen) return DkvForm::Sweep;
  if (b.splits > 1 && !b.varlen) return DkvForm::Waves4;
  const bool narrow = b.D * b.es <= kDkv2WBytes, lean = b.es == 2 && !b.bias && !narrow && b.D * b.es <= 256;
  if (const int env = sweep_env("FCSA_DKV_FORM"); (narrow && bwd_ksplit(b.es, b.D, b.bias)) || lean) {
    if (env == 1) return narrow ? DkvForm::Waves8 : DkvForm::Lean8;
    if (env == 2 && narrow) return DkvForm::QSplit8;
    if (env == 3) return DkvForm::Waves4;
  }
  if (narrow) {
    if (tile_waves(b.batch_heads, b.M, b.causal, b.es == 2, 1, cus) == 8) return DkvForm::Waves8;
    if (bwd_ksplit(b.es, b.D, false) && b.N >= 512 && tile_workgroups(b.batch_heads, b.M, 128, b.causal) <= cus) return DkvForm::QSplit8;
  } else if (lean) {
    if (tile_waves(b.batch_heads, b.M, b.causal, true, 1, cus) == 8) return DkvForm::Lean8;
  }
  return DkvForm::Waves4;
}

struct SplitModel { double tA, cA, tB, cB, tC, cC, a0, b0, k0, k1, alpha; int slabs, extra; };
constexpr SplitModel kSplitFwd = {5.57, 8.68, 3.61, 11.8, 5.77, 16.1, 0.0, 0.536, 7.77, 0.177, 0.585, 1, 1};
constexpr SplitModel kSplitDq  = {11.3, 9.94, 2.35, 12.5, 1.0, 20.9, 0.369, 0.244, 12.2, 0.455, 0.526, 1, 0};
constexpr SplitModel kSplitDkv = {11.5, 12.0, 2.25, 15.5, 1.0, 26.6, 0.11, 0.281, 13.5, 0.34, 0.528, 2, 0};
inline double split_cost(const SplitModel& m, int D, int64_t tiles, int64_t rows, int len, int s, int cus, bool form_a) {
  const bool wide = D * 2 > 128;
  const double ft = m.a0 + (1.0 - m.a0) * D / 64.0, fc = m.b0 + (1.0 - m.b0) * std::max(0.44, D / 64.0);
  const int64_t tot = tiles * s;
  double t0 = m.tA, c = m.cA;
  int64_t slots = cus;
  if (!form_a) {
    if (wide || tot <= cus) { t0 = m.tB; c = m.cB; }
    else { t0 = m.tC; c = m.cC; slots = 2 * (int64_t)cus; }
  }
  const double per = t0 * ft + c * fc * ((double)len / s) / 1024.0;
  const int64_t full = tot / slots, rem = tot % slots;
  const double rounds = full == 0 ? 1.0 : (double)full + (rem == 0 ? 0.0 : m.alpha + (1.0 - m.alpha) * (double)rem / (double)slots);
  const double second = s == 1 ? 0.0 : m.k0 + m.k1 * m.slabs * (double)s * (double)rows * (D + m.extra) * 4.0 / 1e6;
  return rounds * per + second;
}
inline int best_split(const SplitModel& m, bool fwd, int D, int64_t tiles, int64_t rows, int len, int cus) {
  if (tiles <= 0 || tiles >= cus) return 1;
  int best = 1;
  double best_cost = split_cost(m, D, tiles, rows, len, 1, cus, true);
  for (int s = 2; s <= 16 && len / s >= 512; ++s) {
    const bool form_a = fwd && fwd_ksplit(2, D, false) && fwd_ksplit_pays(2, D, tiles * s, cus);
    const double cost = split_cost(m, D, tiles, rows, len, s, cus, form_a);
    if (cost < best_cost) { best_cost = cost; best = s; }
  }
  return best;
}
inline int split_by_target(const fcsa_problem& p, int64_t wgs, int len, int cus) {
  const int target = ((p.dtype == FCSA_F32 ? 4 : 2) * p.dim_head <= 128 ? 2 : 1) * cus;
  if (wgs <= 0 || wgs >= target / 2) return 1;
  int64_t s = (target + wgs - 1) / wgs;
  if (s > 16) s = 16;
  if (s > len / 512) s = len / 512;
  return s >= 2 ? (int)s : 1;
}
inline int sweep_splits(const char* name, int len) {
  const int v = sweep_env(name);
  return v >= 1 ? std::min(std::min(v, 16), std::max(1, len / 64)) : 0;
}

inline int forward_splits(const fcsa_problem& p, bool dyn, int cus) {
  const bool bits16 = p.dtype != FCSA_F32;
  const int64_t bh = (int64_t)p.batch * p.heads, wgs = tile_workgroups(bh, p.q_len, 128, p.causal);
  if (dyn || (p.causal && (!bits16 || p.q_len < 256)) || wgs <= 0) return 1;
  if (const int v = sweep_splits("FCSA_SPLITS", p.k_len)) return v;
  if (bits16) return best_split(kSplitFwd, true, p.dim_head, wgs, bh * p.q_len, p.k_len, cus);
  return split_by_target(p, wgs, p.k_len, cus);
}

inline int backward_dq_splits(const fcsa_problem& p, int cus) {
  const bool bits16 = p.dtype != FCSA_F32;
  if (!p.causal || (bits16 && p.q_len >= 256))
    if (const int v = sweep_splits("FCSA_DQ_SPLITS", p.k_len)) return v;
  if (p.causal && (!bits16 || p.q_len < 256)) return 1;
  const int64_t bh = (int64_t)p.batch * p.heads, wgs = tile_workgroups(bh, p.q_len, 128, p.causal);
  if (bits16) return best_split(kSplitDq, false, p.dim_head, wgs, bh * p.q_len, p.k_len, cus);
  return split_by_target(p, wgs, p.k_len, cus);
}

inline int backward_dkv_splits(const fcsa_problem& p, int cus) {
  const bool bits16 = p.dtype != FCSA_F32;
  if (!p.causal || (bits16 && p.k_len >= 256))
    if (const int v = sweep_splits("FCSA_DKV_SPLITS", p.q_len)) return v;
  if (p.causal && (!bits16 || p.k_len < 256)) return 1;
  const int64_t bh = (int64_t)p.batch * p.heads, wgs = tile_workgroups(bh, p.k_len, 128, p.causal);
  if (bits16) return best_split(kSplitDkv, false, p.dim_head, wgs, bh * p.k_len, p.causal ? std::min(p.q_len, p.k_len) : p.q_len, cus);
  return split_by_target(p, wgs, p.q_len, cus);
}

}
```

flash_cosine_sim_attention_amd/csrc/fcsa_fwd3.hip:

```cpp
#include <cstdlib>
#include <type_traits>
#include <utility>

#include "fcsa_common.cuh"
#include "fcsa_kernels.h"

namespace fcsa {

template <typename F, int... I> FCSA_DEV void static_for_impl(F&& f, std::integer_sequence<int, I...>) { (f(std::integral_constant<int, I>{}), ...); }
template <int N, typename F> FCSA_DEV void static_for(F&& f) { static_for_impl(f, std::make_integer_sequence<int, N>{}); }

template <typename T> struct Ins;
#define FCSA_INS(TYPE, MF, CVT, DOT)                                                                                                  \
  template <> struct Ins<TYPE> {                                                                                                   \
     \
    static FCSA_DEV void s_first(f32x16& d, const u32x4& a, const u32x4& b, const f32x16& c) {                                      \
      asm volatile(MF " %0, %1, %2, %3" : "=&v"(d) : "a"(a), "a"(b), "v"(c));                                                        \
    }                                                                                                                              \
    static FCSA_DEV void s_next(f32x16& d, const u32x4& a, const u32x4& b) { asm volatile(MF " %0, %1, %2, %0" : "+v"(d) : "a"(a), "a"(b)); } \
                                                      \
    static FCSA_DEV void pv(f32x16& d, const u32x4& a, const u32x4& b) { asm volatile(MF " %0, %1, %2, %0" : "+a"(d) : "v"(a), "v"(b)); }    \
    static FCSA_DEV void cvt_pk(uint32_t& d, float a, float b) { asm volatile(CVT " %0, %1, %2" : "=v"(d) : "v"(a), "v"(b)); }              \
                                            \
    static FCSA_DEV void add_pair(float& acc, uint32_t u, uint32_t one2) { asm volatile(DOT " %0, %1, %2" : "+v"(acc) : "v"(u), "v"(one2)); }  \
  }
FCSA_INS(BF16, "v_mfma_f32_32x32x16_bf16", "v_cvt_pk_bf16_f32", "v_dot2c_f32_bf16_e32");
FCSA_INS(F16, "v_mfma_f32_32x32x16_f16", "v_cvt_pk_f16_f32", "v_dot2c_f32_f16_e32");
#undef FCSA_INS

template <int OFF> FCSA_DEV void lds_read_k(u32x4& d, uint32_t addr) { asm volatile("ds_read_b128 %0, %1 offset:%2" : "=a"(d) : "v"(addr), "i"(OFF)); }
template <int OFF, int HALF> FCSA_DEV void lds_read_vt_half(u32x2 (&d)[2], uint32_t a) {
  asm volatile("ds_read_b64_tr_b16 %0, %1 offset:%2" : "=v"(d[HALF]) : "v"(a), "i"(OFF));
}
FCSA_DEV u32x4 vt_frag(const u32x2 (&h)[2]) { u32x4 d; d[0] = h[0][0]; d[1] = h[0][1]; d[2] = h[1][0]; d[3] = h[1][1]; return d; }
template <int N> FCSA_DEV void wait_lgkm() { asm volatile("s_waitcnt lgkmcnt(%0)" :: "n"(N) : "memory"); }
template <int N> FCSA_DEV void wait_vm() { asm volatile("s_waitcnt vmcnt(%0)" :: "n"(N) : "memory"); }
FCSA_DEV void wg_barrier() { asm volatile("s_barrier" ::: "memory"); }

template <typename T> struct F3State {
  f32x16 o[2][4];
  u32x4 q[2][8];
  u32x4 kf[8];
  f32x16 s[2][2];
  u32x4 pk[2][2][2];
  u32x2 vfh[8][2];
  f32x16 cinit;
  float l[2][2];
  float ninf;
  uint32_t one2;
  uint32_t ka[8];
  uint32_t va[8];
};

template <bool MASKED, int R_, int KOFF> FCSA_DEV void sm_exp1(f32x16& s, int thr, float ninf) {
  if constexpr (MASKED) {
    asm volatile("v_cmp_le_i32_e32 vcc, %2, %1\n\tv_cndmask_b32_e32 %0, %3, %0, vcc" : "+v"(s[R_]) : "v"(thr), "n"(KOFF + crow(R_, 0)), "v"(ninf) : "vcc");
  }
  asm volatile("v_exp_f32_e32 %0, %0" : "+v"(s[R_]));
}
template <bool RSUM, int R_> FCSA_DEV void sm_add1(const f32x16& s, float (&l)[2]) {
  if constexpr (!RSUM) asm volatile("v_add_f32_e32 %0, %0, %1" : "+v"(l[R_ & 1]) : "v"(s[R_]));
}
template <typename T, bool RSUM, int E> FCSA_DEV void sm_pack1(const f32x16& s, u32x4 (&pk)[2], float (&l)[2], uint32_t one2) {
  uint32_t u;
  Ins<T>::cvt_pk(u, s[2 * E], s[2 * E + 1]);
  if constexpr (RSUM) Ins<T>::add_pair(l[E & 1], u, one2);
  pk[E >> 2][E & 3] = u;
}
template <typename T, bool RSUM, bool MASKED, int HALF, int G, int KOFF>
FCSA_DEV void sm_gap(F3State<T>& st, f32x16 (&s)[2], u32x4 (&pk)[2][2], const int (&thr)[2]) {
  if constexpr (G >= 1) sm_add1<RSUM, G - 1>(s[HALF], st.l[HALF]);
  sm_exp1<MASKED, G, KOFF>(s[HALF], thr[HALF], st.ninf);
  if constexpr (G >= 2 && (G & 1) == 0) sm_pack1<T, RSUM, (G - 2) / 2>(s[HALF], pk[HALF], st.l[HALF], st.one2);
}
template <typename T, bool RSUM, int HALF>
FCSA_DEV void sm_tail(F3State<T>& st, f32x16 (&s)[2], u32x4 (&pk)[2][2]) {
  sm_add1<RSUM, 15>(s[HALF], st.l[HALF]);
  sm_pack1<T, RSUM, 7>(s[HALF], pk[HALF], st.l[HALF], st.one2);
}

template <int A, int B> constexpr int cmin() { return A < B ? A : B; }
#pragma clang diagnostic push
#pragma clang diagnostic ignored "-Winline-asm"
FCSA_DEV void dma_piece(uint32_t lds_dst, uint32_t voff, const u32x4& rs, uint32_t soff) {
  asm volatile("s_mov_b32 m0, %0\n\ts_nop 0\n\tbuffer_load_dwordx4 %1, %2, %3 offen lds" :: "s"(lds_dst), "v"(voff), "s"(rs), "s"(soff) : "memory", "m0");
}
#pragma clang diagnostic pop
FCSA_DEV void addr_step(uint32_t& a, uint32_t delta) { asm volatile("v_add_u32_e32 %0, %1, %0" : "+v"(a) : "s"(delta)); }

template <typename T, int VOFF, typename Filler, typename Extra>
FCSA_DEV void s_phase(F3State<T>& st, f32x16 (&sblk)[2], Filler&& filler, Extra&& extra) {
  static_for<16>([&](auto gc) {
    constexpr int g = decltype(gc)::value, ks = g >> 1, qb = g & 1;
    if constexpr (qb == 0) wait_lgkm<cmin<15, (7 - ks) + 2 * cmin<g, 8>()>()>();
    if constexpr (ks == 0) Ins<T>::s_first(sblk[qb], st.kf[0], st.q[qb][0], st.cinit);
    else Ins<T>::s_next(sblk[qb], st.kf[ks], st.q[qb][ks]);
    filler(gc);
    if constexpr (g < 8) {
      lds_read_vt_half<VOFF + 16 * (g >> 2) * 256, 0>(st.vfh[g], st.va[2 * (g & 3)]);
      lds_read_vt_half<VOFF + 16 * (g >> 2) * 256, 1>(st.vfh[g], st.va[2 * (g & 3) + 1]);
    }
    extra(gc);
  });
}
template <typename T, int KOFFB, typename Filler, typename Extra>
FCSA_DEV void pv_phase(F3State<T>& st, u32x4 (&pblk)[2][2], Filler&& filler, Extra&& extra) {
  static_for<16>([&](auto gc) {
    constexpr int g = decltype(gc)::value, f = g >> 1, qb = g & 1, ks2 = f >> 2, db = f & 3;
    if constexpr (qb == 0) wait_lgkm<cmin<15, (14 - 2 * f) + cmin<g, 8>()>()>();
    Ins<T>::pv(st.o[qb][db], vt_frag(st.vfh[f]), pblk[qb][ks2]);
    filler(gc);
    if constexpr (g < 8) lds_read_k<KOFFB>(st.kf[g], st.ka[g]);
    extra(gc);
  });
}

template <typename T, int R, bool RSUM, bool MASKED, typename DmaK, typename DmaV>
FCSA_DEV void fwd3_tile(F3State<T>& st, Trace& ts, uint32_t dk_next, uint32_t dv_next, const int (&thr_prev)[2], const int (&thr_cur)[2], DmaK&& dma_k, DmaV&& dma_v) {
  FCSA_STAMP(ts, 0);
  s_phase<T, 8192>(st, st.s[0],
                        [&](auto gc) {
                          constexpr int g = decltype(gc)::value;
                          if constexpr (g == 0) sm_tail<T, RSUM, 0>(st, st.s[1], st.pk[1]);
                          sm_gap<T, RSUM, MASKED, 1, g, 32>(st, st.s[1], st.pk[1], thr_prev);
                        },
                        [&](auto gc) { constexpr int g = decltype(gc)::value; if constexpr (g >= 8) addr_step(st.va[g - 8], dv_next); });
  FCSA_STAMP(ts, 1);
  pv_phase<T, 8192>(st, st.pk[1],
                         [&](auto gc) {
                           constexpr int g = decltype(gc)::value;
                           if constexpr (g == 0) sm_tail<T, RSUM, 1>(st, st.s[1], st.pk[1]);
                           sm_gap<T, RSUM, MASKED, 0, g, 0>(st, st.s[0], st.pk[0], thr_cur);
                         },
                         [&](auto gc) { constexpr int g = decltype(gc)::value; if constexpr (g >= 8 && (g & 1) == 0) dma_k((g - 8) >> 1); });
  FCSA_STAMP(ts, 2);
  wait_lgkm<0>();
  wait_vm<8 * (R - 3) + 4>();
  wg_barrier();
  FCSA_STAMP(ts, 3);
  s_phase<T, 0>(st, st.s[1],
                     [&](auto gc) {
                       constexpr int g = decltype(gc)::value;
                       if constexpr (g == 0) sm_tail<T, RSUM, 0>(st, st.s[0], st.pk[0]);
                       sm_gap<T, RSUM, MASKED, 1, g, 0>(st, st.s[0], st.pk[0], thr_cur);
                     },
                     [&](auto gc) { constexpr int g = decltype(gc)::value; if constexpr (g >= 8) addr_step(st.ka[g - 8], dk_next); });
  FCSA_STAMP(ts, 4);
  pv_phase<T, 0>(st, st.pk[0],
                      [&](auto gc) {
                        constexpr int g = decltype(gc)::value;
                        if constexpr (g == 0) sm_tail<T, RSUM, 1>(st, st.s[0], st.pk[0]);
                        sm_gap<T, RSUM, MASKED, 0, g, 32>(st, st.s[1], st.pk[1], thr_cur);
                      },
                      [&](auto gc) { constexpr int g = decltype(gc)::value; if constexpr (g >= 8 && (g & 1) == 0) dma_v((g - 8) >> 1); });
  FCSA_STAMP(ts, 5);
}

template <typename T, bool RSUM>
FCSA_DEV void fwd3_drain(F3State<T>& st, const int (&thr_last)[2]) {
  static_for<8>([&](auto gc) {
    constexpr int g = decltype(gc)::value;
    lds_read_vt_half<8192 + 16 * (g >> 2) * 256, 0>(st.vfh[g], st.va[2 * (g & 3)]);
    lds_read_vt_half<8192 + 16 * (g >> 2) * 256, 1>(st.vfh[g], st.va[2 * (g & 3) + 1]);
  });
  sm_tail<T, RSUM, 0>(st, st.s[1], st.pk[1]);
  static_for<16>([&](auto gc) {
    sm_gap<T, RSUM, true, 1, decltype(gc)::value, 32>(st, st.s[1], st.pk[1], thr_last);
    asm volatile("s_nop 1");
  });
  asm volatile("s_nop 1");
  sm_tail<T, RSUM, 1>(st, st.s[1], st.pk[1]);
  wait_lgkm<0>();
  asm volatile("s_nop 4");
  static_for<16>([&](auto gc) {
    constexpr int g = decltype(gc)::value, f = g >> 1, qb = g & 1;
    Ins<T>::pv(st.o[qb][f & 3], vt_frag(st.vfh[f]), st.pk[1][qb][f >> 2]);
  });
  asm volatile("s_nop 15\n\ts_nop 15");
}

template <int OFF, bool FIRST> FCSA_DEV void q_load(u32x4& d, uint32_t voff, const u32x4& rs) {
  if constexpr (FIRST) asm volatile("s_nop 4\n\tbuffer_load_dwordx4 %0, %1, %2, 0 offen offset:%3" : "=v"(d) : "v"(voff), "s"(rs), "i"(OFF));
  else asm volatile("buffer_load_dwordx4 %0, %1, %2, 0 offen offset:%3" : "=v"(d) : "v"(voff), "s"(rs), "i"(OFF));
}
template <int N> FCSA_DEV void q_wait(u32x4 (&q)[2][8]) {
  asm volatile("s_waitcnt vmcnt(%8)" : "+v"(q[0][0]), "+v"(q[0][1]), "+v"(q[0][2]), "+v"(q[0][3]), "+v"(q[0][4]), "+v"(q[0][5]), "+v"(q[0][6]), "+v"(q[0][7]) : "n"(N));
  asm volatile("" : "+v"(q[1][0]), "+v"(q[1][1]), "+v"(q[1][2]), "+v"(q[1][3]), "+v"(q[1][4]), "+v"(q[1][5]), "+v"(q[1][6]), "+v"(q[1][7]));
}
FCSA_DEV float xhalf_sum_swap(float x) {
  const uint32_t bits = __builtin_bit_cast(uint32_t, x);
  const auto sw = __builtin_amdgcn_permlane32_swap(bits, bits, false, false);
  return __builtin_bit_cast(float, (uint32_t)sw[0]) + __builtin_bit_cast(float, (uint32_t)sw[1]);
}
template <typename T>
FCSA_DEV void fwd3_finish_q(const FwdParams& p, int b, int h, int i, int hi_, u32x4 (&qf)[8]) {
  constexpr int D = 128;
  if (p.q_raw) {
    float pr[8];
#pragma unroll
    for (int kk = 0; kk < 8; ++kk) {
      const float ss = dot_frag<T>(qf[kk], qf[kk]);
      pr[kk] = p.lgm >= 1 ? xhalf_sum_swap(ss) : ss;
    }
    const int sh = p.lgm >= 1 ? p.lgm - 1 : 0;
    auto rn = [&](float tot) { return 1.f / fmaxf(sqrtf(tot), p.norm_eps); };
    float r[8];
    if (sh >= 3) {
      const float v = rn(((((((pr[0] + pr[1]) + pr[2]) + pr[3]) + pr[4]) + pr[5]) + pr[6]) + pr[7]);
#pragma unroll
      for (int kk = 0; kk < 8; ++kk) r[kk] = v;
    } else if (sh == 2) {
      const float v0 = rn(((pr[0] + pr[1]) + pr[2]) + pr[3]), v1 = rn(((pr[4] + pr[5]) + pr[6]) + pr[7]);
#pragma unroll
      for (int kk = 0; kk < 8; ++kk) r[kk] = kk < 4 ? v0 : v1;
    } else if (sh == 1) {
#pragma unroll
      for (int g = 0; g < 4; ++g) { const float v = rn(pr[2 * g] + pr[2 * g + 1]); r[2 * g] = v; r[2 * g + 1] = v; }
    } else {
#pragma unroll
      for (int kk = 0; kk < 8; ++kk) r[kk] = rn(pr[kk]);
    }
    const int64_t row = ((int64_t)b * p.H + h) * p.N + i;
#pragma unroll
    for (int kk = 0; kk < 8; ++kk) {
      qf[kk] = scale_frag<T>(qf[kk], r[kk] * p.c1);
      if (i < p.N) {
        const int c = 2 * kk + hi_;
        if (p.qn_out != nullptr) *reinterpret_cast<u32x4*>(p.qn_out + (row * D + 8 * c) * 2) = qf[kk];
        if (p.rq_out != nullptr && (c & ((1 << p.lgm) - 1)) == 0) p.rq_out[row * p.G + (c >> p.lgm)] = r[kk];
      }
    }
    return;
  }
  if (!p.q_scaled) {
#pragma unroll
    for (int kk = 0; kk < 8; ++kk) qf[kk] = scale_frag<T>(qf[kk], p.c1);
  }
}

FCSA_TRACE_PHASE_SITE(fwd3)

template <typename T, int R> struct Fwd3Lds {
  static constexpr int TILE_B = 64 * TileGeom<128, 2>::ROWB;
  static constexpr int EPI_B = RowEpilogue<T, 128>::BYTES_NOX;
  static constexpr int TOTAL = lds_max(2 * R * TILE_B, 4 * EPI_B);
  static_assert(TILE_B == 16384 && TOTAL <= kLdsBytes, "fwd3_kernel LDS");
};

template <typename T, int R, bool RSUM>
__global__ void __launch_bounds__(256, 1) fwd3_kernel(const FwdParams p) {
  constexpr int D = 128;
  typedef DmaStager<T, D, 64, 4> DS;
  typedef Fwd3Lds<T, R> LDS;
  constexpr int BN = 64, RW = 64, NW = 4, BM = RW * NW;
  constexpr int TILE_B = LDS::TILE_B;
  static_assert(DS::PER == 4 && DS::UNIFORM && R >= 3, "fwd3 geometry");
  extern __shared__ __attribute__((aligned(16))) char smem[];

  const int tid = threadIdx.x;
  const int lane = tid & 63;
  const int wave = __builtin_amdgcn_readfirstlane(tid >> 6);
  FragAddr<T, D> fa;
  fa.init(lane);
  const uint32_t lds0 = DS::lds_addr(smem);

  const int MT = tile_count(p.N, BM), PT = tile_pairs(MT, p.causal);
  int bh, pt;
  block_work(blockIdx.x, p.B * p.H, PT, bh, pt);
  const int b = bh / p.H, h = bh % p.H;
  const int npass = pair_passes(MT, pt, p.causal);
  const int diff = p.M - p.N;
  const int hk = h / p.kv_group;
  const char* kbase = p.k.p + (int64_t)b * p.k.sb + (int64_t)hk * p.k.sh;
  const char* vbase = p.v.p + (int64_t)b * p.v.sb + (int64_t)hk * p.v.sh;
  DS dk_, dv_;
  dk_.init(p.k.sn, wave, lane);
  dv_.init(p.v.sn, wave, lane);
  const uint32_t k_step = (uint32_t)(BN * p.k.sn), v_step = (uint32_t)(BN * p.v.sn);

  Trace ts;
  ts.reset();
  TraceRec<TraceSite_fwd3, kTracePhase, 8> tr;
  tr.start();
  F3State<T> st;
  {
    float c0 = -p.c2;
    asm volatile("" : "+v"(c0));
#pragma unroll
    for (int e = 0; e < 16; ++e) st.cinit[e] = c0;
    float ni = -INFINITY;
    asm volatile("" : "+v"(ni));
    st.ninf = ni;
    uint32_t o2 = Traits<T>::kOne2;
    asm volatile("" : "+v"(o2));
    st.one2 = o2;
  }
  for (int pass = 0; pass < npass; ++pass) {
    const int m0 = pass_tile(MT, pt, pass, p.causal, true) * BM;
    const int mw = m0 + wave * RW;
    const int i0 = mw + (lane & 31);
    const int nt = key_tiles(p.M, m0, BM, diff, p.causal, BN);

    tr.mark(pass, 0);
    u32x4 qf[2][8];
    {
      const char* qbase = p.q.p + (int64_t)b * p.q.sb + (int64_t)h * p.q.sh;
      int64_t qbytes = (int64_t)(p.N - 1) * p.q.sn + D * 2;
      if (qbytes > 0x7fffffff) qbytes = 0x7fffffff;
      const uint64_t qa = reinterpret_cast<uint64_t>(qbase);
      u32x4 qrs;
      qrs[0] = __builtin_amdgcn_readfirstlane((uint32_t)qa);
      qrs[1] = __builtin_amdgcn_readfirstlane((uint32_t)(qa >> 32) & 0xffffu);
      qrs[2] = __builtin_amdgcn_readfirstlane((uint32_t)qbytes);
      qrs[3] = 0x00020000u;
      const int hio = opaque(fa.hi);
      const uint32_t qv0 = (uint32_t)i0 * (uint32_t)p.q.sn + (uint32_t)hio * 16u, qv1 = qv0 + 32u * (uint32_t)p.q.sn;
      static_for<8>([&](auto kc) { constexpr int kk = decltype(kc)::value; q_load<32 * kk, kk == 0>(qf[0][kk], qv0, qrs); });
      static_for<8>([&](auto kc) { constexpr int kk = decltype(kc)::value; q_load<32 * kk, false>(qf[1][kk], qv1, qrs); });
    }
    typename DS::Stream stk = dk_.open(kbase, p.k.sn, p.M), stv = dv_.open(vbase, p.v.sn, p.M);
    {
      const typename DS::Stream stz = dv_.open(vbase, p.v.sn, 0);
      dv_.issue(stz, lds0 + (2 * R - 1) * TILE_B, wave);
      dk_.issue(stk, lds0, wave);
      stk.off += k_step;
      dv_.issue(stv, lds0 + R * TILE_B, wave);
      stv.off += v_step;
    }
    tr.mark(pass, 1);
    u32x4 krs, vrs;
#pragma unroll
    for (int e = 0; e < 4; ++e) { krs[e] = __builtin_amdgcn_readfirstlane(stk.rs[e]); vrs[e] = __builtin_amdgcn_readfirstlane(stv.rs[e]); }
    q_wait<12>(qf);
    {
      const int hio = opaque(fa.hi);
      fwd3_finish_q<T>(p, b, h, i0, hio, qf[0]);
#pragma unroll
      for (int s = 1; s < R - 1; ++s) {
        dk_.issue(stk, lds0 + s * TILE_B, wave);
        stk.off += k_step;
        if (s < R - 2) {
          dv_.issue(stv, lds0 + (R + s) * TILE_B, wave);
          stv.off += v_step;
        }
      }
      fwd3_finish_q<T>(p, b, h, i0 + 32, hio, qf[1]);
    }
    tr.mark(pass, 2);
#pragma unroll
    for (int r = 0; r < 2; ++r)
#pragma unroll
      for (int kk = 0; kk < 8; ++kk) asm volatile("" : "=a"(st.q[r][kk]) : "0"(qf[r][kk]));
    {
      f32x16 z;
#pragma unroll
      for (int e = 0; e < 16; ++e) z[e] = 0.f;
#pragma unroll
      for (int r = 0; r < 2; ++r)
#pragma unroll
        for (int db = 0; db < 4; ++db) asm volatile("" : "=a"(st.o[r][db]) : "0"(z));
    }
#pragma unroll
    for (int r = 0; r < 2; ++r) {
#pragma unroll
      for (int e = 0; e < 16; ++e) st.s[1][r][e] = r == 0 ? 0.f : -1e30f;
      const u32x4 z4 = {0u, 0u, 0u, 0u};
      st.pk[1][r][0] = z4;
      st.pk[1][r][1] = z4;
      st.l[r][0] = 0.f;
      st.l[r][1] = 0.f;
    }
#pragma unroll
    for (int kk = 0; kk < 8; ++kk) st.ka[kk] = lds0 + fa.row_off + (((2 * kk + fa.hi) ^ fa.row_swz) << 4);
#pragma unroll
    for (int db = 0; db < 4; ++db)
#pragma unroll
      for (int half = 0; half < 2; ++half)
        st.va[2 * db + half] = lds0 + (2 * R - 1) * TILE_B + fa.tr_off[half] + (((4 * db + fa.tr_col) ^ fa.tr_swz[half]) << 4);
    tr.mark(pass, 3);
    wait_vm<0>();
    wg_barrier();
    tr.mark(pass, 4);
    static_for<8>([&](auto kc) { lds_read_k<0>(st.kf[decltype(kc)::value], st.ka[decltype(kc)::value]); });

    int thr0[2];
#pragma unroll
    for (int r = 0; r < 2; ++r) thr0[r] = (p.causal ? min(i0 + 32 * r + diff, p.M - 1) : p.M - 1) - 4 * fa.hi;
    int t_split = p.M / BN;
    if (p.causal) t_split = min(t_split, max(0, mw + diff + 1) / BN);
    t_split = min(t_split, nt);

// ... 79 lines not shown
```

flash_cosine_sim_attention_amd/csrc/fcsa_kernels.h:

```cpp
#pragma once
#include <hip/hip_runtime.h>
#include <stdint.h>
#include <atomic>

#include "fcsa_dispatch.h"

namespace fcsa {

struct View {
  char*   p;
  int64_t sb, sh, sn;
};

struct SeqTable {
  const int32_t* cu_q;
  const int32_t* cu_k;
  int total_q, total_k;
};

struct FwdParams {
  View q, k, v, o;
  float* inv_l;
  const uint8_t* mask;
  const char* bias;
  int B, H, N, M;
  int kv_group;
  int causal, bias_batch;
  float c1;
  float c2;
  float bias_c;
  float l_eps;
  int q_scaled;
  int dyn;
  int q_raw;
  char* qn_out;
  float* rq_out;
  int G, lgm;
  float norm_eps;
  int splits;
  float* ws_o;
  float* ws_l;
  SeqTable seq;
};
struct FwdWinParams : FwdParams {
  int window = 0;
  int win_lo = 0, win_hi = 0;
};

struct BwdParams {
  View q, k, v, o, d_out;
  View dq;
  View dk, dv;
  int dq_f32, dk_f32, dv_f32;
  const float* inv_l;
  int invl_log2;
  float* delta;
  const uint8_t* mask;
  const char* bias;
  void* d_bias;
  int dq_splits;
  int64_t dq_split_stride;
  int dkv_splits;
  int64_t dkv_split_stride;
  int B, H, N, M;
  int kv_group;
  int kv_sweep;
  int causal, bias_batch;
  float c1, c2, bias_c;
  float scale;
  int q_scaled;
  const float* rq;
  const float* rk;
  int G, lgm;
  float norm_eps;
  SeqTable seq;
  const float* dlse = nullptr;
};
struct BwdWinParams : BwdParams {
  int window = 0;
  int win_lo = 0, win_hi = 0;
};

struct NormParams {
  View x;
  char* xn;
  float* inv_norm;
  int B, H, L, D, G;
  float eps;
  float out_scale;
};

struct NormBwdParams {
  const char* slab;
  int slab_f32;
  int HS;
  const char* xn;
  const float* inv_norm;
  View dx;
  int B, HO, L, D, G;
  float eps;
  float xn_scale;
};

struct DecodeParams {
  View q, o;
  View kc, vc;
  View kn, vn;
  const int32_t* seqlens;
  const int32_t* table;
  int64_t table_stride;
  int capacity, page, num_blocks, new_len;
  int B, H, Hk, G, N;
  int row_tiles, splits;
  int causal, l2norm, groups;
  float c1;
  float c2;
  float l_eps;
  int dyn;
  float* ws_o;
  float* ws_ml;
};
struct DecodeWinParams : DecodeParams {
  int window = 0;
  int win_lo = 0, win_hi = 0;
};
struct DecodeFp8Params : DecodeWinParams {
  const float* k_scale = nullptr;
  const float* v_scale = nullptr;
  int64_t ks_b = 0, ks_h = 0, vs_b = 0, vs_h = 0;
};
struct DecodeRaggedParams : DecodeFp8Params {
  const int32_t* cu_q = nullptr;
  int total_q = 0;
  int slots = 0;
  int append = 0;
};
struct DecodeLseOut {
  float*  lse;
  int64_t sb, sh, sn;
};
struct DecodeTreeMask {
  const uint64_t* words;
};
struct DecodeAlibi {
  const float* slopes;
  int64_t sb, sh;
};
struct DecodeStepParams : DecodeRaggedParams {
  int chunk_rows = 0;
};
struct DecodeForm { bool fp8, ragged, step; };
hipError_t launch_kv_append(int dtype, int D, DecodeForm f, const DecodeStepParams& p, hipStream_t s);
hipError_t launch_decode(int dtype, int D, DecodeForm f, const DecodeStepParams& p, hipStream_t s);
hipError_t launch_decode_combine(int dtype, int D, DecodeForm f, const DecodeStepParams& p, const DecodeLseOut* lse, hipStream_t s);
hipError_t launch_decode_tree(int dtype, int D, DecodeForm f, const DecodeStepParams& p, const DecodeTreeMask& tree, hipStream_t s);
constexpr int kCompactSlots = 64;
struct CompactParams {
  const int32_t* accepted;
  const int32_t* num_accepted;
  int64_t accepted_stride;
  int A;
  int row_bytes;
};
hipError_t launch_kv_compact(const DecodeParams& cache, const CompactParams& c, hipStream_t s);
hipError_t launch_prefill(int dtype, int D, DecodeForm f, const DecodeStepParams& p, const DecodeLseOut* lse, hipStream_t s);
hipError_t launch_decode_alibi(int dtype, int D, DecodeForm f, const DecodeStepParams& p, const DecodeAlibi& alibi, hipStream_t s);
hipError_t launch_prefill_alibi(int dtype, int D, DecodeForm f, const DecodeStepParams& p, const DecodeAlibi& alibi, const DecodeLseOut* lse, hipStream_t s);

struct MergeParams {
  View         o_in[8];
  DecodeLseOut lse_in[8];
  View         o;
  DecodeLseOut lse;
  int n0, n1, n2, D, S;
};
hipError_t launch_merge_states(int dtype, const MergeParams& p, hipStream_t s);
struct MergeBwdParams {
  View         o_in[8];
  DecodeLseOut lse_in[8];
  View         d_o;
  DecodeLseOut d_lse;
  View         d_o_in[8];
  DecodeLseOut d_lse_in[8];
  int n0, n1, n2, D, S;
};
hipError_t launch_merge_states_backward(int dtype, const MergeBwdParams& p, hipStream_t s);

struct StateLseParams {
  const float* inv_l;
  DecodeLseOut out;
  int B, H, N, M;
  int win_lo, win_hi;
  float c2;
  int invl_log2;
  SeqTable seq;
};
hipError_t launch_state_lse(const StateLseParams& p, hipStream_t s);

template <typename K>
static inline hipError_t ensure_dynamic_lds(K kern, size_t lds, std::atomic<uint64_t>& done) {
  int dev = 0;
  if (hipError_t e = hipGetDevice(&dev); e != hipSuccess) return e;
  const uint64_t bit = (dev >= 0 && dev < 64) ? (1ull << dev) : 0ull;
  if (bit != 0 && (done.load(std::memory_order_acquire) & bit) != 0) return hipSuccess;
  const hipError_t e = hipFuncSetAttribute(reinterpret_cast<const void*>(kern), hipFuncAttributeMaxDynamicSharedMemorySize, (int)lds);
  if (e == hipSuccess && bit != 0) done.fetch_or(bit, std::memory_order_release);
  return e;
}

template <auto Kernel, typename... Args>
static inline hipError_t launch_with_lds(dim3 grid, dim3 block, size_t lds, hipStream_t s, const Args&... args) {
  static std::atomic<uint64_t> done{0};
  if (hipError_t e = ensure_dynamic_lds(Kernel, lds, done); e != hipSuccess) return e;
  hipLaunchKernelGGL(Kernel, grid, block, lds, s, args...);
  return hipGetLastError();
}

inline int cu_count() {
  static std::atomic<int> cached[64];
  int dev = 0, cus = 0;
  if (hipGetDevice(&dev) != hipSuccess) {
    (void)hipGetLastError();
    return 256;
  }
  const bool slot = dev >= 0 && dev < 64;
  if (slot) {
    const int n = cached[dev].load(std::memory_order_relaxed);
    if (n > 0) return n;
  }
  if (hipDeviceGetAttribute(&cus, hipDeviceAttributeMultiprocessorCount, dev) != hipSuccess || cus <= 0) {
    (void)hipGetLastError();
    return 256;
  }
  if (slot) cached[dev].store(cus, std::memory_order_relaxed);
  return cus;
}

hipError_t launch_forward(int dtype, int D, const FwdWinParams& p, hipStream_t s);
int forward_wide128_mode(int set);
hipError_t launch_forward_wide128(int dtype, const FwdParams& p, hipStream_t s);
hipError_t launch_backward_dq(int dtype, int D, const BwdWinParams& p, hipStream_t s);
hipError_t launch_backward_dbias(int dtype, int D, const BwdParams& p, hipStream_t s);
hipError_t launch_backward_dkv(int dtype, int D, const BwdWinParams& p, hipStream_t s);
int kv_group_mode(int set);
hipError_t launch_l2norm(int dtype, const NormParams& p, hipStream_t s);
hipError_t launch_l2norm_pair(int dtype, const NormParams& a, const NormParams& b, hipStream_t s);
hipError_t launch_l2norm_bwd(int dtype, const NormBwdParams& p, hipStream_t s);
hipError_t launch_l2norm_bwd_pair(int dtype, const NormBwdParams& a, const NormBwdParams& b, hipStream_t s);
hipError_t launch_l2norm_bwd_triple(int dtype, const NormBwdParams& a, const NormBwdParams& b, const NormBwdParams& c, hipStream_t s);

}
```

include/fcsa.h:

```cpp
#ifndef FCSA_H_
#define FCSA_H_

#include <stddef.h>
#include <stdint.h>

#ifdef __cplusplus
extern "C" {
#endif

#define FCSA_ABI_VERSION 4

enum fcsa_status {
  FCSA_OK = 0,
  FCSA_ERR_INVALID_ARG = -1,
  FCSA_ERR_UNSUPPORTED = -2,
  FCSA_ERR_LAUNCH = -3,
  FCSA_ERR_WORKSPACE = -4
};

enum fcsa_dtype {
  FCSA_F32 = 0,
  FCSA_F16 = 1,
  FCSA_BF16 = 2
};

typedef struct fcsa_tensor {
  void*   ptr;
  int64_t stride0;
  int64_t stride1;
  int64_t stride2;
} fcsa_tensor;

typedef struct fcsa_problem {
  int32_t dtype;
  int32_t batch;
  int32_t heads;
  int32_t kv_heads;
  int32_t q_len;
  int32_t k_len;
  int32_t dim_head;
  int32_t causal;
  int32_t bias_batch_dim;
  int32_t l2norm_qk;
  int32_t groups;
  float   scale;
} fcsa_problem;

typedef struct fcsa_norm_state {
  void*  qn;
  void*  kn;
  float* rq;
  float* rk;
} fcsa_norm_state;

typedef struct fcsa_forward_args {
  fcsa_problem    p;
  fcsa_tensor     q, k, v;
  fcsa_tensor     o;
  float*          inv_l;
  const uint8_t*  mask;
  const void*     attn_bias;
  fcsa_norm_state norm;
  void*           workspace;
  size_t          workspace_bytes;
  void*           stream;
} fcsa_forward_args;

typedef struct fcsa_backward_args {
  fcsa_problem    p;
  fcsa_tensor     d_out, o;
  const float*    inv_l;
  fcsa_tensor     q, k, v;
  const uint8_t*  mask;
  const void*     attn_bias;
  fcsa_norm_state norm;
  fcsa_tensor     dq;
  fcsa_tensor     dk, dv;
  void*           d_bias;
  void*           workspace;
  size_t          workspace_bytes;
  void*           stream;
} fcsa_backward_args;

int fcsa_forward(const fcsa_forward_args* args);

int fcsa_backward(const fcsa_backward_args* args);

size_t fcsa_backward_workspace_bytes(const fcsa_problem* p);

typedef struct fcsa_varlen {
  const int32_t* cu_seqlens_q;
  const int32_t* cu_seqlens_k;
  int64_t total_q, total_k;
} fcsa_varlen;
int    fcsa_forward_varlen(const fcsa_forward_args* args, const fcsa_varlen* seqs);
int    fcsa_backward_varlen(const fcsa_backward_args* args, const fcsa_varlen* seqs);
size_t fcsa_backward_varlen_workspace_bytes(const fcsa_problem* p, const fcsa_varlen* seqs);

typedef struct fcsa_kvcache {
  fcsa_tensor    k_cache, v_cache;
  int32_t        capacity;
  int32_t        page_size;
  int32_t        num_blocks;
  int32_t        new_len;
  const int32_t* cache_seqlens;
  const int32_t* block_table;
  int64_t        block_table_stride;
  fcsa_tensor    k_new, v_new;
} fcsa_kvcache;
int    fcsa_forward_kvcache(const fcsa_forward_args* args, const fcsa_kvcache* cache);
size_t fcsa_forward_kvcache_workspace_bytes(const fcsa_problem* p, const fcsa_kvcache* cache);

typedef struct fcsa_window {
  int32_t left, right;
} fcsa_window;
int    fcsa_forward_window(const fcsa_forward_args* args, const fcsa_varlen* seqs, const fcsa_window* window);
int    fcsa_backward_window(const fcsa_backward_args* args, const fcsa_varlen* seqs, const fcsa_window* window);
size_t fcsa_backward_window_workspace_bytes(const fcsa_problem* p, const fcsa_varlen* seqs, const fcsa_window* window);
int    fcsa_forward_kvcache_window(const fcsa_forward_args* args, const fcsa_kvcache* cache, const fcsa_window* window);
size_t fcsa_forward_kvcache_window_workspace_bytes(const fcsa_problem* p, const fcsa_kvcache* cache, const fcsa_window* window);

#define FCSA_CACHE_E4M3 1
typedef struct fcsa_kvcache_quant {
  int32_t      cache_dtype;
  const float* k_scale;
  const float* v_scale;
  int64_t      k_scale_stride0, k_scale_stride1;
  int64_t      v_scale_stride0, v_scale_stride1;
} fcsa_kvcache_quant;
int    fcsa_forward_kvcache_quant(const fcsa_forward_args* args, const fcsa_kvcache* cache, const fcsa_kvcache_quant* quant,
                                  const fcsa_window* window);
size_t fcsa_forward_kvcache_quant_workspace_bytes(const fcsa_problem* p, const fcsa_kvcache* cache, const fcsa_kvcache_quant* quant,
                                                  const fcsa_window* window);

int    fcsa_forward_kvcache_varlen(const fcsa_forward_args* args, const fcsa_kvcache* cache, const fcsa_varlen* seqs,
                                   const fcsa_kvcache_quant* quant, const fcsa_window* window);
size_t fcsa_forward_kvcache_varlen_workspace_bytes(const fcsa_problem* p, const fcsa_kvcache* cache, const fcsa_varlen* seqs,
                                                   const fcsa_kvcache_quant* quant, const fcsa_window* window);

typedef struct fcsa_lse_out {
  float*  lse;
  int64_t stride0;
  int64_t stride1;
  int64_t stride2;
} fcsa_lse_out;
int    fcsa_forward_kvcache_lse(const fcsa_forward_args* args, const fcsa_kvcache* cache, const fcsa_varlen* seqs,
                                const fcsa_kvcache_quant* quant, const fcsa_window* window, const fcsa_lse_out* lse_out);

int    fcsa_forward_kvcache_prefill(const fcsa_forward_args* args, const fcsa_kvcache* cache, const fcsa_varlen* seqs,
                                    const fcsa_lse_out* lse_out);

#define FCSA_STEP_CHUNK_ROWS 1024
typedef struct fcsa_kvcache_step {
  int32_t chunk_rows;
  int32_t no_decode;
  int64_t max_decode_tokens;
  int32_t no_chunk;
  int32_t reserved;
} fcsa_kvcache_step;
int    fcsa_forward_kvcache_step(const fcsa_forward_args* args, const fcsa_kvcache* cache, const fcsa_varlen* seqs,
                                 const fcsa_kvcache_quant* quant, const fcsa_window* window, const fcsa_kvcache_step* step,
                                 const fcsa_lse_out* lse_out);
size_t fcsa_forward_kvcache_step_workspace_bytes(const fcsa_problem* p, const fcsa_kvcache* cache, const fcsa_varlen* seqs,
                                                 const fcsa_kvcache_quant* quant, const fcsa_window* window,
                                                 const fcsa_kvcache_step* step);

typedef struct fcsa_tree_mask {
  const uint64_t* mask;
  int64_t         reserved;
} fcsa_tree_mask;
int    fcsa_forward_kvcache_tree(const fcsa_forward_args* args, const fcsa_kvcache* cache, const fcsa_varlen* seqs,
                                 const fcsa_kvcache_quant* quant, const fcsa_tree_mask* tree, const fcsa_lse_out* lse_out);

typedef struct fcsa_alibi {
  const float* slopes;
  int64_t      stride_b;
  int64_t      stride_h;
  int64_t      reserved;
} fcsa_alibi;
int    fcsa_forward_kvcache_alibi(const fcsa_forward_args* args, const fcsa_kvcache* cache, const fcsa_varlen* seqs,
                                  const fcsa_kvcache_quant* quant, const fcsa_window* window, const fcsa_kvcache_step* step,
                                  const fcsa_alibi* alibi, const fcsa_lse_out* lse_out);

int    fcsa_kvcache_compact(const fcsa_kvcache* cache, int32_t batch, int32_t kv_heads, int32_t dim_head, int32_t elem_bytes,
                            const int32_t* accepted, int64_t accepted_stride, int32_t max_accepted, const int32_t* num_accepted,
                            void* stream);

#define FCSA_MERGE_MAX_STATES 8
typedef struct fcsa_merge_args {
  int32_t      dtype;
  int32_t      size0, size1, size2;
  int32_t      dim_head;
  int32_t      states;
  fcsa_tensor  o_in[8];
  fcsa_lse_out lse_in[8];
  fcsa_tensor  o;
  fcsa_lse_out lse;
  void*        stream;
} fcsa_merge_args;
int    fcsa_merge_states(const fcsa_merge_args* args);

int    fcsa_attention_lse(const fcsa_problem* p, const float* inv_l, const fcsa_varlen* seqs, const fcsa_window* window,
                          const fcsa_lse_out* lse_out, void* stream);
int    fcsa_backward_state(const fcsa_backward_args* args, const fcsa_varlen* seqs, const fcsa_window* window, const float* d_lse);

typedef struct fcsa_merge_backward_args {
  int32_t      dtype;
  int32_t      size0, size1, size2;
  int32_t      dim_head;
  int32_t      states;
  fcsa_tensor  o_in[8];
  fcsa_lse_out lse_in[8];
  fcsa_tensor  d_o;
  fcsa_lse_out d_lse;
  fcsa_tensor  d_o_in[8];
  fcsa_lse_out d_lse_in[8];
  void*        stream;
} fcsa_merge_backward_args;
int    fcsa_merge_states_backward(const fcsa_merge_backward_args* args);

size_t fcsa_forward_workspace_bytes(const fcsa_problem* p);

int fcsa_forward_needs_qn(const fcsa_problem* p, int32_t need_backward);

int fcsa_l2norm(int32_t dtype, int32_t batch, int32_t heads, int32_t len, int32_t dim_head, int32_t groups,
                const fcsa_tensor* x, void* xn, float* inv_norm, void* stream);

int fcsa_debug(char* buf, size_t buf_bytes);

typedef struct fcsa_kernel_stat {
  char    name[32];
  int32_t calls;
  float   total_ms;
  float   min_ms;
  float   max_ms;
} fcsa_kernel_stat;
int fcsa_profile_enable(int32_t enable);
int fcsa_profile_collect(fcsa_kernel_stat* stats, int32_t capacity);

int fcsa_debug_forward_form(int32_t form);

int fcsa_debug_kv_group_form(int32_t form);

const char* fcsa_last_error(void);

#ifdef __cplusplus
}
#endif
#endif
```

Baseline: 764.8.

## Add hand-scheduled asm dQ backward kernel for causal bf16 D=64

Adds a new dQ backward kernel for causal, equal-length, D=64, 16-bit problems. It streams K/V tiles into a 4-slot LDS ring with buffer_load-to-LDS DMA and interleaves the S, dP and dQ MFMA phases with the exp, multiply and pack work in hand-written inline asm. The dispatcher picks it by default when the existing choice would be Waves8 and the grid is large enough, and it also forces dQ splits to 1 in mode 2. Shared asm helpers are moved out of the forward kernel into a common header. The aim is better MFMA utilisation and overlap of memory with compute in the dQ pass, at the cost of a large, fragile asm schedule.

```diff
diff --git a/flash_cosine_sim_attention_amd/_lib.py b/flash_cosine_sim_attention_amd/_lib.py
--- a/flash_cosine_sim_attention_amd/_lib.py
+++ b/flash_cosine_sim_attention_amd/_lib.py
@@ -78,7 +78,7 @@
 
 
 EXPORTS = ("fcsa_forward", "fcsa_backward", "fcsa_backward_workspace_bytes", "fcsa_forward_workspace_bytes", "fcsa_forward_needs_qn",
-           "fcsa_l2norm", "fcsa_debug", "fcsa_debug_forward_form", "fcsa_debug_kv_group_form", "fcsa_last_error", "fcsa_profile_enable", "fcsa_profile_collect",
+           "fcsa_l2norm", "fcsa_debug", "fcsa_debug_forward_form", "fcsa_debug_kv_group_form", "fcsa_debug_dq_form", "fcsa_last_error", "fcsa_profile_enable", "fcsa_profile_collect",
            "fcsa_forward_varlen", "fcsa_backward_varlen", "fcsa_backward_varlen_workspace_bytes", "fcsa_forward_kvcache",
            "fcsa_forward_kvcache_workspace_bytes", "fcsa_forward_window", "fcsa_backward_window", "fcsa_backward_window_workspace_bytes",
            "fcsa_forward_kvcache_window", "fcsa_forward_kvcache_window_workspace_bytes", "fcsa_forward_kvcache_quant",
@@ -131,6 +131,9 @@
     lib.fcsa_debug_forward_form.restype = C.c_int
     lib.fcsa_debug_kv_group_form.argtypes = [C.c_int32]
     lib.fcsa_debug_kv_group_form.restype = C.c_int
+    if hasattr(lib, "fcsa_debug_dq_form"):
+        lib.fcsa_debug_dq_form.argtypes = [C.c_int32]
+        lib.fcsa_debug_dq_form.restype = C.c_int
     lib.fcsa_profile_enable.argtypes = [C.c_int32]
     lib.fcsa_profile_enable.restype = C.c_int
     lib.fcsa_profile_collect.argtypes = [C.POINTER(KernelStat), C.c_int32]
@@ -226,6 +229,10 @@
     return int(load().fcsa_debug_kv_group_form(int(form)))
 
 
+def dq_form(form: int) -> int:
+    return int(load().fcsa_debug_dq_form(int(form)))
+
+
 def source_sha256() -> str:
     import hashlib
     h = hashlib.sha256()
diff --git a/flash_cosine_sim_attention_amd/csrc/fcsa_asm.cuh b/flash_cosine_sim_attention_amd/csrc/fcsa_asm.cuh
--- /dev/null
+++ b/flash_cosine_sim_attention_amd/csrc/fcsa_asm.cuh
@@ -0,0 +1,46 @@
+#pragma once
+#include <type_traits>
+#include <utility>
+
+#include "fcsa_common.cuh"
+
+namespace fcsa {
+
+template <typename F, int... I> FCSA_DEV void static_for_impl(F&& f, std::integer_sequence<int, I...>) { (f(std::integral_constant<int, I>{}), ...); }
+template <int N, typename F> FCSA_DEV void static_for(F&& f) { static_for_impl(f, std::make_integer_sequence<int, N>{}); }
+
+template <typename T> struct Ins;
+#define FCSA_INS(TYPE, MF, CVT, DOT)                                                                                                  \
+  template <> struct Ins<TYPE> {                                                                                                   \
+     \
+    static FCSA_DEV void s_first(f32x16& d, const u32x4& a, const u32x4& b, const f32x16& c) {                                      \
+      asm volatile(MF " %0, %1, %2, %3" : "=&v"(d) : "a"(a), "a"(b), "v"(c));                                                        \
+    }                                                                                                                              \
+    static FCSA_DEV void s_next(f32x16& d, const u32x4& a, const u32x4& b) { asm volatile(MF " %0, %1, %2, %0" : "+v"(d) : "a"(a), "a"(b)); } \
+                                                      \
+    static FCSA_DEV void pv(f32x16& d, const u32x4& a, const u32x4& b) { asm volatile(MF " %0, %1, %2, %0" : "+a"(d) : "v"(a), "v"(b)); }    \
+                                                    \
+    static FCSA_DEV void acc_av(f32x16& d, const u32x4& a, const u32x4& b) { asm volatile(MF " %0, %1, %2, %0" : "+a"(d) : "a"(a), "v"(b)); } \
+    static FCSA_DEV void cvt_pk(uint32_t& d, float a, float b) { asm volatile(CVT " %0, %1, %2" : "=v"(d) : "v"(a), "v"(b)); }              \
+                                            \
+    static FCSA_DEV void add_pair(float& acc, uint32_t u, uint32_t one2) { asm volatile(DOT " %0, %1, %2" : "+v"(acc) : "v"(u), "v"(one2)); }  \
+  }
+FCSA_INS(BF16, "v_mfma_f32_32x32x16_bf16", "v_cvt_pk_bf16_f32", "v_dot2c_f32_bf16_e32");
+FCSA_INS(F16, "v_mfma_f32_32x32x16_f16", "v_cvt_pk_f16_f32", "v_dot2c_f32_f16_e32");
+#undef FCSA_INS
+
+template <int OFF> FCSA_DEV void lds_read_k(u32x4& d, uint32_t addr) { asm volatile("ds_read_b128 %0, %1 offset:%2" : "=a"(d) : "v"(addr), "i"(OFF)); }
+template <int N> FCSA_DEV void wait_lgkm() { asm volatile("s_waitcnt lgkmcnt(%0)" :: "n"(N) : "memory"); }
+template <int N> FCSA_DEV void wait_vm() { asm volatile("s_waitcnt vmcnt(%0)" :: "n"(N) : "memory"); }
+FCSA_DEV void wg_barrier() { asm volatile("s_barrier" ::: "memory"); }
+
+template <int A, int B> constexpr int cmin() { return A < B ? A : B; }
+#pragma clang diagnostic push
+#pragma clang diagnostic ignored "-Winline-asm"
+FCSA_DEV void dma_piece(uint32_t lds_dst, uint32_t voff, const u32x4& rs, uint32_t soff) {
+  asm volatile("s_mov_b32 m0, %0\n\ts_nop 0\n\tbuffer_load_dwordx4 %1, %2, %3 offen lds" :: "s"(lds_dst), "v"(voff), "s"(rs), "s"(soff) : "memory", "m0");
+}
+#pragma clang diagnostic pop
+FCSA_DEV void addr_step(uint32_t& a, uint32_t delta) { asm volatile("v_add_u32_e32 %0, %1, %0" : "+v"(a) : "s"(delta)); }
+
+}
diff --git a/flash_cosine_sim_attention_amd/csrc/fcsa_bwd.hip b/flash_cosine_sim_attention_amd/csrc/fcsa_bwd.hip
--- a/flash_cosine_sim_attention_amd/csrc/fcsa_bwd.hip
+++ b/flash_cosine_sim_attention_amd/csrc/fcsa_bwd.hip
@@ -1481,8 +1481,12 @@
 }
 
 static BwdProblem bwd_problem(int dtype, int D, const BwdWinParams& p, int splits) {
-  return {dtype == 0 ? 4 : 2, D, (int64_t)p.B * p.H, p.N, p.M, p.causal != 0, p.bias != nullptr, splits, p.kv_sweep != 0,
-          p.seq.cu_q != nullptr || p.window != 0, p.window != 0};
+  BwdProblem b{dtype == 0 ? 4 : 2, D, (int64_t)p.B * p.H, p.N, p.M, p.causal != 0, p.bias != nullptr, splits, p.kv_sweep != 0,
+               p.seq.cu_q != nullptr || p.window != 0, p.window != 0};
+  b.mask = p.mask != nullptr;
+  b.kv_offsets32 = (int64_t)(p.M + kDq3Ahead) * p.k.sn < 0x7fffffffLL && (int64_t)(p.M + kDq3Ahead) * p.v.sn < 0x7fffffffLL;
+  b.dq_form_mode = dq_rows64_mode(-1);
+  return b;
 }
 
 hipError_t launch_backward_dbias(int dtype, int D, const BwdParams& p, hipStream_t s) {
@@ -1492,7 +1496,9 @@
 
 hipError_t launch_backward_dq(int dtype, int D, const BwdWinParams& p, hipStream_t s) {
   if (p.B * p.H == 0 || p.N == 0) return hipSuccess;
-  const DqForm f = choose_dq(bwd_problem(dtype, D, p, p.dq_splits), cu_count());
+  const BwdProblem pb = bwd_problem(dtype, D, p, p.dq_splits);
+  if (dq_rows64_applies(pb, cu_count())) return launch_backward_dq_rows64(dtype, p, s);
+  const DqForm f = choose_dq(pb, cu_count());
   return dispatch_dtype_d(dtype, D, [&](auto td) {
     using T = typename decltype(td)::T;
     constexpr int DD = decltype(td)::D;
diff --git a/flash_cosine_sim_attention_amd/csrc/fcsa_capi.hip b/flash_cosine_sim_attention_amd/csrc/fcsa_capi.hip
--- a/flash_cosine_sim_attention_amd/csrc/fcsa_capi.hip
+++ b/flash_cosine_sim_attention_amd/csrc/fcsa_capi.hip
@@ -137,7 +137,7 @@
   b.kv_sweep = sweep && call != nullptr && !call->bias;
   b.fuse_norm = p.l2norm_qk != 0 && fusable_groups(p);
   const bool norm_slab = p.l2norm_qk != 0 && !b.fuse_norm;
-  b.dq_splits = varlen || (call != nullptr && !(call->dq_flat && !(p.causal && call->bias))) ? 1 : fcsa::backward_dq_splits(p, cus);
+  b.dq_splits = varlen || (call != nullptr && !(call->dq_flat && !(p.causal && call->bias))) ? 1 : fcsa::backward_dq_splits(p, cus, fcsa::dq_rows64_mode(-1));
   b.dkv_splits = varlen || sweep || (call != nullptr && !((call->dkv_flat || grouped) && !call->bias)) ? 1 : fcsa::backward_dkv_splits(p, cus);
   b.dq_slab = b.dq_splits > 1 || norm_slab;
   b.dk_slab = !b.kv_sweep && (b.dkv_splits > 1 || grouped || norm_slab);
@@ -280,6 +280,8 @@
 int fcsa_debug_forward_form(int32_t form) { return fcsa::forward_wide128_mode(form); }
 
 int fcsa_debug_kv_group_form(int32_t form) { return fcsa::kv_group_mode(form); }
+
+int fcsa_debug_dq_form(int32_t form) { return fcsa::dq_rows64_mode(form); }
 
 int fcsa_l2norm(int32_t dtype, int32_t batch, int32_t heads, int32_t len, int32_t dim_head, int32_t groups,
                 const fcsa_tensor* x, void* xn, float* inv_norm, void* stream) {
diff --git a/flash_cosine_sim_attention_amd/csrc/fcsa_dispatch.h b/flash_cosine_sim_attention_amd/csrc/fcsa_dispatch.h
--- a/flash_cosine_sim_attention_amd/csrc/fcsa_dispatch.h
+++ b/flash_cosine_sim_attention_amd/csrc/fcsa_dispatch.h
@@ -331,7 +331,18 @@
   bool kv_sweep;
   bool varlen = false;
   bool window = false;
+  bool mask = false;
+  bool kv_offsets32 = false;
+  int dq_form_mode = 0;
 };
+
+constexpr int kDq3Ahead = 64 * 6;
+inline bool dq_rows64_valid(const BwdProblem& b) {
+  return b.es == 2 && b.D == 64 && b.causal && !b.varlen && !b.window && b.N == b.M && !b.bias && !b.mask && b.splits <= 1 && b.kv_offsets32;
+}
+inline bool dq_rows64_pays(const BwdProblem& b, int cus) {
+  return b.N >= 4096 && b.batch_heads * tile_pairs(tile_count(b.N, 256), 1) >= (int64_t)cus * 7 / 8;
+}
 
 inline DqForm choose_dq(const BwdProblem& b, int cus) {
   if (b.splits > 1 && !b.varlen) return DqForm::Waves4;
@@ -351,6 +362,11 @@
     if (bwd_ksplit(b.es, b.D, b.bias) && b.causal) return DqForm::KSplit8;
   }
   return DqForm::Waves4;
+}
+
+inline bool dq_rows64_applies(const BwdProblem& b, int cus) {
+  if (b.dq_form_mode <= 0 || !dq_rows64_valid(b)) return false;
+  return b.dq_form_mode >= 2 || (choose_dq(b, cus) == DqForm::Waves8 && dq_rows64_pays(b, cus));
 }
 
 inline bool dkv_sweep(int es, int D, int64_t batch_kv_heads, int M, bool causal, int mode, int cus) {
@@ -429,8 +445,9 @@
   return split_by_target(p, wgs, p.k_len, cus);
 }
 
-inline int backward_dq_splits(const fcsa_problem& p, int cus) {
+inline int backward_dq_splits(const fcsa_problem& p, int cus, int dq_form_mode = 1) {
   const bool bits16 = p.dtype != FCSA_F32;
+  if (dq_form_mode >= 2 && bits16 && p.dim_head == 64 && p.causal && p.q_len == p.k_len) return 1;
   if (!p.causal || (bits16 && p.q_len >= 256))
     if (const int v = sweep_splits("FCSA_DQ_SPLITS", p.k_len)) return v;
   if (p.causal && (!bits16 || p.q_len < 256)) return 1;
diff --git a/flash_cosine_sim_attention_amd/csrc/fcsa_dq3.hip b/flash_cosine_sim_attention_amd/csrc/fcsa_dq3.hip
--- /dev/null
+++ b/flash_cosine_sim_attention_amd/csrc/fcsa_dq3.hip
@@ -0,0 +1,403 @@
+#include <cstdlib>
+
+#include "fcsa_asm.cuh"
+#include "fcsa_kernels.h"
+
+namespace fcsa {
+
+FCSA_TRACE_SITE(dq3)
+
+template <int OFF, int HALF> FCSA_DEV void lds_read_kt_half(u32x2 (&d)[2], uint32_t a) {
+  asm volatile("ds_read_b64_tr_b16 %0, %1 offset:%2" : "=v"(d[HALF]) : "v"(a), "i"(OFF));
+}
+FCSA_DEV u32x4 kt_frag(const u32x2 (&h)[2]) { u32x4 d; d[0] = h[0][0]; d[1] = h[0][1]; d[2] = h[1][0]; d[3] = h[1][1]; return d; }
+
+template <typename T> struct Dq3State {
+  f32x16 dq[2][2];
+  u32x4 q[2][4];
+  u32x4 dof[2][4];
+  u32x4 kf[4];
+  u32x4 vf[4];
+  u32x2 kth[4][2];
+  f32x16 s[2][2];
+  f32x16 dp[2];
+  u32x4 pk[2][2][2];
+  f32x16 clc[2];
+  f32x16 cnd[2];
+  float ninf;
+  uint32_t ka[4];
+  uint32_t kta[4];
+};
+
+template <bool MASKED, int R_, int KOFF> FCSA_DEV void dq3_exp1(f32x16& s, int thr, float ninf) {
+  if constexpr (MASKED) {
+    asm volatile("v_cmp_le_i32_e32 vcc, %2, %1\n\tv_cndmask_b32_e32 %0, %3, %0, vcc" : "+v"(s[R_]) : "v"(thr), "n"(KOFF + crow(R_, 0)), "v"(ninf) : "vcc");
+  }
+  asm volatile("v_exp_f32_e32 %0, %0" : "+v"(s[R_]));
+}
+template <int R_> FCSA_DEV void dq3_mul1(f32x16& s, const f32x16& dp) { asm volatile("v_mul_f32_e32 %0, %0, %1" : "+v"(s[R_]) : "v"(dp[R_])); }
+template <typename T, int E> FCSA_DEV void dq3_pack1(const f32x16& s, u32x4 (&pk)[2]) {
+  uint32_t u;
+  Ins<T>::cvt_pk(u, s[2 * E], s[2 * E + 1]);
+  pk[E >> 2][E & 3] = u;
+}
+template <bool MASKED, int G, int KOFF> FCSA_DEV void dq3_exp_gap(f32x16& s, int thr, float ninf) {
+  dq3_exp1<MASKED, 2 * G, KOFF>(s, thr, ninf);
+  dq3_exp1<MASKED, 2 * G + 1, KOFF>(s, thr, ninf);
+}
+template <typename T, int G> FCSA_DEV void dq3_ds_gap(f32x16& s, const f32x16& dp, u32x4 (&pk)[2]) {
+  dq3_mul1<2 * G>(s, dp);
+  dq3_mul1<2 * G + 1>(s, dp);
+  if constexpr (G >= 1) dq3_pack1<T, G - 1>(s, pk);
+}
+template <typename T> FCSA_DEV void dq3_pack_tail(const f32x16& s, u32x4 (&pk)[2]) { dq3_pack1<T, 7>(s, pk); }
+
+template <typename T, int VOFF, typename Filler, typename Extra>
+FCSA_DEV void dq3_s_phase(Dq3State<T>& st, f32x16 (&sblk)[2], Filler&& filler, Extra&& extra) {
+  static_for<8>([&](auto gc) {
+    constexpr int g = decltype(gc)::value, ks = g >> 1, qb = g & 1;
+    if constexpr (qb == 0) wait_lgkm<(3 - ks) + cmin<g, 4>()>();
+    if constexpr (ks == 0) Ins<T>::s_first(sblk[qb], st.kf[0], st.q[qb][0], st.clc[qb]);
+    else Ins<T>::s_next(sblk[qb], st.kf[ks], st.q[qb][ks]);
+    filler(gc);
+    if constexpr (g < 4) lds_read_k<VOFF>(st.vf[g], st.ka[g]);
+    extra(gc);
+  });
+}
+template <typename T, int KTOFF, typename Filler, typename Extra>
+FCSA_DEV void dq3_dp_phase(Dq3State<T>& st, Filler&& filler, Extra&& extra) {
+  static_for<8>([&](auto gc) {
+    constexpr int g = decltype(gc)::value, ks = g >> 1, qb = g & 1;
+    if constexpr (qb == 0) wait_lgkm<(3 - ks) + 2 * cmin<g, 4>()>();
+    if constexpr (ks == 0) Ins<T>::s_first(st.dp[qb], st.vf[0], st.dof[qb][0], st.cnd[qb]);
+    else Ins<T>::s_next(st.dp[qb], st.vf[ks], st.dof[qb][ks]);
+    filler(gc);
+    if constexpr (g < 4) {
+      lds_read_kt_half<KTOFF + (g >> 1) * 2048, 0>(st.kth[g], st.kta[2 * (g & 1)]);
+      lds_read_kt_half<KTOFF + (g >> 1) * 2048, 1>(st.kth[g], st.kta[2 * (g & 1) + 1]);
+    }
+    extra(gc);
+  });
+}
+template <typename T, int KOFF, typename Filler, typename Extra>
+FCSA_DEV void dq3_dq_phase(Dq3State<T>& st, u32x4 (&pblk)[2][2], Filler&& filler, Extra&& extra) {
+  static_for<8>([&](auto gc) {
+    constexpr int g = decltype(gc)::value, f = g >> 1, qb = g & 1, ks2 = f >> 1, db = f & 1;
+    if constexpr (qb == 0) wait_lgkm<(6 - 2 * f) + cmin<g, 4>()>();
+    Ins<T>::pv(st.dq[qb][db], kt_frag(st.kth[f]), pblk[qb][ks2]);
+    filler(gc);
+    if constexpr (g < 4) lds_read_k<KOFF>(st.kf[g], st.ka[g]);
+    extra(gc);
+  });
+}
+
+constexpr int kDq3TileB = 16384;
+
+template <typename T, int R, bool MASKED, typename DmaK, typename DmaV>
+FCSA_DEV void dq3_tile(Dq3State<T>& st, Trace& ts, uint32_t dka_next, uint32_t dkta_next, const int (&thr)[2], DmaK&& dma_k, DmaV&& dma_v) {
+  auto none = [](auto) {};
+  FCSA_STAMP(ts, 0);
+  dq3_s_phase<T, 8192>(st, st.s[0],
+                       [&](auto gc) {
+                         constexpr int g = decltype(gc)::value;
+                         if constexpr (g == 0) dq3_pack_tail<T>(st.s[1][0], st.pk[1][0]);
+                         dq3_ds_gap<T, g>(st.s[1][1], st.dp[1], st.pk[1][1]);
+                       },
+                       none);
+  FCSA_STAMP(ts, 1);
+  dq3_dp_phase<T, 4096>(st,
+                        [&](auto gc) {
+                          constexpr int g = decltype(gc)::value;
+                          if constexpr (g == 0) dq3_pack_tail<T>(st.s[1][1], st.pk[1][1]);
+                          dq3_exp_gap<MASKED, g, 0>(st.s[0][0], thr[0], st.ninf);
+                        },
+                        none);
+  FCSA_STAMP(ts, 2);
+  dq3_dq_phase<T, 4096>(st, st.pk[1],
+                        [&](auto gc) {
+                          constexpr int g = decltype(gc)::value;
+                          dq3_exp_gap<MASKED, g, 0>(st.s[0][1], thr[1], st.ninf);
+                          dq3_ds_gap<T, g>(st.s[0][0], st.dp[0], st.pk[0][0]);
+                        },
+                        none);
+  FCSA_STAMP(ts, 3);
+  wait_lgkm<0>();
+  wait_vm<4 * (R - 3)>();
+  wg_barrier();
+  FCSA_STAMP(ts, 4);
+  dq3_s_phase<T, 8192 + 4096>(st, st.s[1],
+                              [&](auto gc) {
+                                constexpr int g = decltype(gc)::value;
+                                if constexpr (g == 0) dq3_pack_tail<T>(st.s[0][0], st.pk[0][0]);
+                                dq3_ds_gap<T, g>(st.s[0][1], st.dp[1], st.pk[0][1]);
+                              },
+                              [&](auto gc) {
+                                constexpr int g = decltype(gc)::value;
+                                if constexpr (g >= 4) addr_step(st.kta[g - 4], dkta_next);
+                                if constexpr (g == 4 || g == 6) dma_k((g - 4) >> 1);
+                              });
+  FCSA_STAMP(ts, 5);
+  dq3_dp_phase<T, 0>(st,
+                     [&](auto gc) {
+                       constexpr int g = decltype(gc)::value;
+                       if constexpr (g == 0) dq3_pack_tail<T>(st.s[0][1], st.pk[0][1]);
+                       dq3_exp_gap<MASKED, g, 32>(st.s[1][0], thr[0], st.ninf);
+                     },
+                     [&](auto gc) { constexpr int g = decltype(gc)::value; if constexpr (g >= 4) addr_step(st.ka[g - 4], dka_next); });
+  FCSA_STAMP(ts, 6);
+  dq3_dq_phase<T, 0>(st, st.pk[0],
+                     [&](auto gc) {
+                       constexpr int g = decltype(gc)::value;
+                       dq3_exp_gap<MASKED, g, 32>(st.s[1][1], thr[1], st.ninf);
+                       dq3_ds_gap<T, g>(st.s[1][0], st.dp[0], st.pk[1][0]);
+                     },
+                     [&](auto gc) { constexpr int g = decltype(gc)::value; if constexpr (g == 4 || g == 6) dma_v((g - 4) >> 1); });
+  FCSA_STAMP(ts, 7);
+}
+
+template <typename T>
+FCSA_DEV void dq3_drain(Dq3State<T>& st) {
+  static_for<4>([&](auto gc) {
+    constexpr int g = decltype(gc)::value;
+    lds_read_kt_half<4096 + (g >> 1) * 2048, 0>(st.kth[g], st.kta[2 * (g & 1)]);
+    lds_read_kt_half<4096 + (g >> 1) * 2048, 1>(st.kth[g], st.kta[2 * (g & 1) + 1]);
+  });
+  asm volatile("s_nop 15\n\ts_nop 15");
+  dq3_pack_tail<T>(st.s[1][0], st.pk[1][0]);
+  static_for<8>([&](auto gc) { dq3_ds_gap<T, decltype(gc)::value>(st.s[1][1], st.dp[1], st.pk[1][1]); });
+  dq3_pack_tail<T>(st.s[1][1], st.pk[1][1]);
+  wait_lgkm<0>();
+  asm volatile("s_nop 4");
+  static_for<8>([&](auto gc) {
+    constexpr int g = decltype(gc)::value, f = g >> 1, qb = g & 1;
+    Ins<T>::pv(st.dq[qb][f & 1], kt_frag(st.kth[f]), st.pk[1][qb][f >> 1]);
+  });
+  asm volatile("s_nop 15\n\ts_nop 15");
+}
+
+template <typename T, int R> struct Dq3Lds {
+  static constexpr int TILE_B = kDq3TileB;
+  static constexpr int EPI_B = RowEpilogue<T, 64>::BYTES;
+  static constexpr int TOTAL = lds_max(R * TILE_B, 4 * EPI_B);
+  static_assert(2 * 64 * TileGeom<64, 2>::ROWB == TILE_B && TOTAL <= kLdsBytes, "bwd_dq3_kernel LDS");
+};
+
+template <typename T, int R>
+__global__ void __launch_bounds__(256, 1) bwd_dq3_kernel(const BwdParams p) {
+  constexpr int D = 64;
+  typedef TileGeom<D, 2> G;
+  typedef DmaStager<T, D, 64, 4> DS;
+  typedef RowEpilogue<T, D> EP;
+  typedef Dq3Lds<T, R> LDS;
+  constexpr int BN = 64, RW = 64, NW = 4, BM = RW * NW;
+  constexpr int TILE_B = LDS::TILE_B, VPART = 64 * G::ROWB;
+  static_assert(DS::PER == 2 && DS::UNIFORM && R >= 3 && G::KS == 4 && G::DB == 2 && VPART == 8192, "dq3 geometry");
+  extern __shared__ __attribute__((aligned(16))) char smem[];
+
+  const int tid = threadIdx.x;
+  const int lane = tid & 63;
+  const int wave = __builtin_amdgcn_readfirstlane(tid >> 6);
+  FragAddr<T, D> fa;
+  fa.init(lane);
+  const uint32_t lds0 = DS::lds_addr(smem);
+
+  const int MT = tile_count(p.N, BM), PT = tile_pairs(MT, 1);
+  int bh, pt;
+  block_work(blockIdx.x, p.B * p.H, PT, bh, pt);
+  const int b = bh / p.H, h = bh % p.H;
+  const int npass = pair_passes(MT, pt, 1);
+  const int diff = p.M - p.N;
+  const int hk = h / p.kv_group;
+  const char* kbase = p.k.p + (int64_t)b * p.k.sb + (int64_t)hk * p.k.sh;
+  const char* vbase = p.v.p + (int64_t)b * p.v.sb + (int64_t)hk * p.v.sh;
+  DS dk_, dv_;
+  dk_.init(p.k.sn, wave, lane);
+  dv_.init(p.v.sn, wave, lane);
+  const uint32_t k_step = (uint32_t)(BN * p.k.sn), v_step = (uint32_t)(BN * p.v.sn);
+
+  Trace ts;
+  ts.reset();
+  TraceRec<TraceSite_dq3> tr;
+  tr.start();
+  Dq3State<T> st;
+  {
+    float ni = -INFINITY;
+    asm volatile("" : "+v"(ni));
+    st.ninf = ni;
+  }
+  for (int pass = 0; pass < npass; ++pass) {
+    const int m0 = pass_tile(MT, pt, pass, 1, true) * BM;
+    const int mw = m0 + wave * RW;
+    const int nt = key_tiles(p.M, m0, BM, diff, 1, BN);
+
+    tr.mark(pass, 0);
+    typename DS::Stream stk = dk_.open(kbase, p.k.sn, p.M), stv = dv_.open(vbase, p.v.sn, p.M);
+    {
+      const typename DS::Stream stz = dk_.open(kbase, p.k.sn, 0);
+      dk_.issue(stz, lds0 + (R - 1) * TILE_B, wave);
+#pragma unroll
+      for (int s = 0; s < R - 1; ++s) {
+        dk_.issue(stk, lds0 + s * TILE_B, wave);
+        stk.off += k_step;
+        dv_.issue(stv, lds0 + s * TILE_B + VPART, wave);
+        stv.off += v_step;
+      }
+    }
+    u32x4 krs, vrs;
+#pragma unroll
+    for (int e = 0; e < 4; ++e) { krs[e] = __builtin_amdgcn_readfirstlane(stk.rs[e]); vrs[e] = __builtin_amdgcn_readfirstlane(stv.rs[e]); }
+
+    u32x4 qf[2][4], dof[2][4];
+    float lcs[2], nds[2];
+#pragma unroll
+    for (int r = 0; r < 2; ++r) {
+      const int ln = opaque(lane), hi_ = ln >> 5;
+      const int i = mw + 32 * r + (ln & 31);
+      const char* qrow = p.q.p + (int64_t)b * p.q.sb + (int64_t)h * p.q.sh + (int64_t)i * p.q.sn;
+      const char* dorow = p.d_out.p + (int64_t)b * p.d_out.sb + (int64_t)h * p.d_out.sh + (int64_t)i * p.d_out.sn;
+      const char* orow = p.o.p + (int64_t)b * p.o.sb + (int64_t)h * p.o.sh + (int64_t)i * p.o.sn;
+      float delta = 0.f, lc = 0.f;
+#pragma unroll
+      for (int kk = 0; kk < G::KS; ++kk) {
+        u32x4 z = {0u, 0u, 0u, 0u};
+        qf[r][kk] = z;
+        dof[r][kk] = z;
+        if (i < p.N) {
+          qf[r][kk] = *reinterpret_cast<const u32x4*>(qrow + (2 * kk + hi_) * 16);
+          if (!p.q_scaled) qf[r][kk] = scale_frag<T>(qf[r][kk], p.c1);
+          dof[r][kk] = *reinterpret_cast<const u32x4*>(dorow + (2 * kk + hi_) * 16);
+          const u32x4 of = *reinterpret_cast<const u32x4*>(orow + (2 * kk + hi_) * 16);
+          delta += dot_frag<T>(dof[r][kk], of);
+        }
+      }
+      const float rinvl = i < p.N ? p.inv_l[((int64_t)b * p.H + h) * p.N + i] : 1.f;
+      delta = xhalf_sum(delta);
+      if (p.dlse != nullptr && i < p.N) delta -= p.dlse[((int64_t)b * p.H + h) * p.N + i];
+      if (i < p.N) {
+        const int64_t ridx = ((int64_t)b * p.H + h) * p.N + i;
+        lc = (p.invl_log2 ? rinvl : __builtin_amdgcn_logf(rinvl)) - p.c2;
+        if (hi_ == 0) p.delta[ridx] = delta;
+      }
+      lcs[r] = lc;
+      nds[r] = -delta;
+    }
+    tr.mark(pass, 1);
+#pragma unroll
+    for (int r = 0; r < 2; ++r) {
+#pragma unroll
+      for (int kk = 0; kk < 4; ++kk) {
+        asm volatile("" : "=a"(st.q[r][kk]) : "0"(qf[r][kk]));
+        asm volatile("" : "=a"(st.dof[r][kk]) : "0"(dof[r][kk]));
+      }
+      float l = lcs[r], d = nds[r];
+      asm volatile("" : "+v"(l));
+      asm volatile("" : "+v"(d));
+#pragma unroll
+      for (int e = 0; e < 16; ++e) { st.clc[r][e] = l; st.cnd[r][e] = d; }
+      asm volatile("" : "+v"(st.clc[r]));
+      asm volatile("" : "+v"(st.cnd[r]));
+    }
+    {
+      f32x16 z;
+#pragma unroll
+      for (int e = 0; e < 16; ++e) z[e] = 0.f;
+#pragma unroll
+      for (int r = 0; r < 2; ++r)
+#pragma unroll
+        for (int db = 0; db < 2; ++db) asm volatile("" : "=a"(st.dq[r][db]) : "0"(z));
+      const u32x4 z4 = {0u, 0u, 0u, 0u};
+#pragma unroll
+      for (int r = 0; r < 2; ++r) {
+        st.s[1][r] = z;
+        st.dp[r] = z;
+#pragma unroll
+        for (int kb = 0; kb < 2; ++kb) { st.pk[kb][r][0] = z4; st.pk[kb][r][1] = z4; }
+      }
+    }
+#pragma unroll
+    for (int kk = 0; kk < 4; ++kk) st.ka[kk] = lds0 + fa.row_off + (((2 * kk + fa.hi) ^ fa.row_swz) << 4);
+#pragma unroll
+    for (int db = 0; db < 2; ++db)
+#pragma unroll
+      for (int half = 0; half < 2; ++half)
+        st.kta[2 * db + half] = lds0 + (R - 1) * TILE_B + fa.tr_off[half] + (((4 * db + fa.tr_col) ^ fa.tr_swz[half]) << 4);
+    wait_vm<0>();
+    wg_barrier();
+    static_for<4>([&](auto kc) { lds_read_k<0>(st.kf[decltype(kc)::value], st.ka[decltype(kc)::value]); });
+
+    int thr0[2];
+#pragma unroll
+    for (int r = 0; r < 2; ++r) thr0[r] = min(mw + 32 * r + (lane & 31) + diff, p.M - 1) - 4 * fa.hi;
+    int t_split = min(p.M / BN, max(0, mw + diff + 1) / BN);
+    t_split = min(t_split, nt);
+
+    int slot = 0;
+    auto run = [&](auto masked_tag, int t_begin, int t_end) {
+      constexpr bool MASKED = decltype(masked_tag)::value;
+      for (int t = t_begin; t < t_end; ++t) {
+        const int sm1 = slot == 0 ? R - 1 : slot - 1;
+        const uint32_t lds_k = lds0 + (uint32_t)sm1 * TILE_B + (uint32_t)wave * 1024u;
+        auto dma_k = [&](int i) { dma_piece(lds_k + (uint32_t)i * 4096u, (uint32_t)dk_.piece_offset(i), krs, stk.off); };
+        auto dma_v = [&](int i) { dma_piece(lds_k + (uint32_t)VPART + (uint32_t)i * 4096u, (uint32_t)dv_.piece_offset(i), vrs, stv.off); };
+        const uint32_t dka_next = slot + 1 == R ? (uint32_t)(-(R - 1) * TILE_B) : (uint32_t)TILE_B;
+        const uint32_t dkta_next = slot == 0 ? (uint32_t)(-(R - 1) * TILE_B) : (uint32_t)TILE_B;
+        const int j0 = t * BN;
+        const int thr[2] = {thr0[0] - j0, thr0[1] - j0};
+        dq3_tile<T, R, MASKED>(st, ts, dka_next, dkta_next, thr, dma_k, dma_v);
+        if constexpr (!MASKED) ts.close(7);
+        stk.off += k_step;
+        stv.off += v_step;
+        slot = slot + 1 == R ? 0 : slot + 1;
+      }
+    };
+    run(std::false_type{}, 0, t_split);
+    tr.mark(pass, 2);
+    run(std::true_type{}, t_split, nt);
+    dq3_drain<T>(st);
+    tr.mark(pass, 3);
+    wait_lgkm<0>();
+    wait_vm<0>();
+    wg_barrier();
+
+    char* scr = smem + wave * LDS::EPI_B;
+    const bool fused = p.rq != nullptr;
+#pragma unroll
+    for (int r = 0; r < 2; ++r) {
+      const int mr = mw + 32 * r;
+      const int rows_valid = p.N - mr;
+      if (rows_valid > 0) {
+        char* dq0 = p.dq.p + (int64_t)b * p.dq.sb + (int64_t)h * p.dq.sh + (int64_t)mr * p.dq.sn;
+        const char* x0 = fused ? p.q.p + (int64_t)b * p.q.sb + (int64_t)h * p.q.sh + (int64_t)mr * p.q.sn : nullptr;
+        const float* rq0 = fused ? p.rq + (((int64_t)b * p.H + h) * p.N + mr) * p.G : nullptr;
+        EP::store(scr, st.dq[r], p.scale, opaque(lane), dq0, p.dq.sn, rows_valid, fused ? false : p.dq_f32 != 0, x0, p.q.sn,
+                  p.q_scaled ? 1.f / p.c1 : 1.f, rq0, p.G, p.lgm, p.norm_eps, fused ? st.q[r] : nullptr);
+      }
+    }
+    tr.mark(pass, 4);
+    if (pass + 1 < npass) {
+      asm volatile("s_waitcnt lgkmcnt(0)" ::: "memory");
+      wg_barrier();
+    }
+  }
+  tr.finish(ts, wave, true, wave);
+}
+
+constexpr int kDq3Ring = 4;
+
+template <typename T>
+static hipError_t launch_dq3_t(const BwdParams& p, hipStream_t s) {
+  return launch_with_lds<bwd_dq3_kernel<T, kDq3Ring>>(dim3((unsigned)((int64_t)p.B * p.H * tile_pairs(tile_count(p.N, 256), 1))), dim3(256),
+                                                      Dq3Lds<T, kDq3Ring>::TOTAL, s, p);
+}
+
+static std::atomic<int> g_dq_rows64{1};
+int dq_rows64_mode(int set) {
+  return set < 0 ? g_dq_rows64.load(std::memory_order_relaxed) : g_dq_rows64.exchange(set > 2 ? 2 : set, std::memory_order_relaxed);
+}
+
+hipError_t launch_backward_dq_rows64(int dtype, const BwdParams& p, hipStream_t s) {
+  if (!p.causal || p.N != p.M || p.bias != nullptr || p.mask != nullptr || p.dq_splits > 1 || p.seq.cu_q != nullptr) return hipErrorInvalidValue;
+  return dtype == 2 ? launch_dq3_t<BF16>(p, s) : dtype == 1 ? launch_dq3_t<F16>(p, s) : hipErrorInvalidValue;
+}
+
+}
diff --git a/flash_cosine_sim_attention_amd/csrc/fcsa_fwd3.hip b/flash_cosine_sim_attention_amd/csrc/fcsa_fwd3.hip
--- a/flash_cosine_sim_attention_amd/csrc/fcsa_fwd3.hip
+++ b/flash_cosine_sim_attention_amd/csrc/fcsa_fwd3.hip
@@ -2,40 +2,15 @@
 #include <type_traits>
 #include <utility>
 
-#include "fcsa_common.cuh"
+#include "fcsa_asm.cuh"
 #include "fcsa_kernels.h"
 
 namespace fcsa {
 
-template <typename F, int... I> FCSA_DEV void static_for_impl(F&& f, std::integer_sequence<int, I...>) { (f(std::integral_constant<int, I>{}), ...); }
-template <int N, typename F> FCSA_DEV void static_for(F&& f) { static_for_impl(f, std::make_integer_sequence<int, N>{}); }
-
-template <typename T> struct Ins;
-#define FCSA_INS(TYPE, MF, CVT, DOT)                                                                                                  \
-  template <> struct Ins<TYPE> {                                                                                                   \
-     \
-    static FCSA_DEV void s_first(f32x16& d, const u32x4& a, const u32x4& b, const f32x16& c) {                                      \
-      asm volatile(MF " %0, %1, %2, %3" : "=&v"(d) : "a"(a), "a"(b), "v"(c));                                                        \
-    }                                                                                                                              \
-    static FCSA_DEV void s_next(f32x16& d, const u32x4& a, const u32x4& b) { asm volatile(MF " %0, %1, %2, %0" : "+v"(d) : "a"(a), "a"(b)); } \
-                                                      \
-    static FCSA_DEV void pv(f32x16& d, const u32x4& a, const u32x4& b) { asm volatile(MF " %0, %1, %2, %0" : "+a"(d) : "v"(a), "v"(b)); }    \
-    static FCSA_DEV void cvt_pk(uint32_t& d, float a, float b) { asm volatile(CVT " %0, %1, %2" : "=v"(d) : "v"(a), "v"(b)); }              \
-                                            \
-    static FCSA_DEV void add_pair(float& acc, uint32_t u, uint32_t one2) { asm volatile(DOT " %0, %1, %2" : "+v"(acc) : "v"(u), "v"(one2)); }  \
-  }
-FCSA_INS(BF16, "v_mfma_f32_32x32x16_bf16", "v_cvt_pk_bf16_f32", "v_dot2c_f32_bf16_e32");
-FCSA_INS(F16, "v_mfma_f32_32x32x16_f16", "v_cvt_pk_f16_f32", "v_dot2c_f32_f16_e32");
-#undef FCSA_INS
-
-template <int OFF> FCSA_DEV void lds_read_k(u32x4& d, uint32_t addr) { asm volatile("ds_read_b128 %0, %1 offset:%2" : "=a"(d) : "v"(addr), "i"(OFF)); }
 template <int OFF, int HALF> FCSA_DEV void lds_read_vt_half(u32x2 (&d)[2], uint32_t a) {
   asm volatile("ds_read_b64_tr_b16 %0, %1 offset:%2" : "=v"(d[HALF]) : "v"(a), "i"(OFF));
 }
 FCSA_DEV u32x4 vt_frag(const u32x2 (&h)[2]) { u32x4 d; d[0] = h[0][0]; d[1] = h[0][1]; d[2] = h[1][0]; d[3] = h[1][1]; return d; }
-template <int N> FCSA_DEV void wait_lgkm() { asm volatile("s_waitcnt lgkmcnt(%0)" :: "n"(N) : "memory"); }
-template <int N> FCSA_DEV void wait_vm() { asm volatile("s_waitcnt vmcnt(%0)" :: "n"(N) : "memory"); }
-FCSA_DEV void wg_barrier() { asm volatile("s_barrier" ::: "memory"); }
 
 template <typename T> struct F3State {
   f32x16 o[2][4];
@@ -79,14 +54,6 @@
   sm_pack1<T, RSUM, 7>(s[HALF], pk[HALF], st.l[HALF], st.one2);
 }
 
-template <int A, int B> constexpr int cmin() { return A < B ? A : B; }
-#pragma clang diagnostic push
-#pragma clang diagnostic ignored "-Winline-asm"
-FCSA_DEV void dma_piece(uint32_t lds_dst, uint32_t voff, const u32x4& rs, uint32_t soff) {
-  asm volatile("s_mov_b32 m0, %0\n\ts_nop 0\n\tbuffer_load_dwordx4 %1, %2, %3 offen lds" :: "s"(lds_dst), "v"(voff), "s"(rs), "s"(soff) : "memory", "m0");
-}
-#pragma clang diagnostic pop
-FCSA_DEV void addr_step(uint32_t& a, uint32_t delta) { asm volatile("v_add_u32_e32 %0, %1, %0" : "+v"(a) : "s"(delta)); }
 
 template <typename T, int VOFF, typename Filler, typename Extra>
 FCSA_DEV void s_phase(F3State<T>& st, f32x16 (&sblk)[2], Filler&& filler, Extra&& extra) {
diff --git a/flash_cosine_sim_attention_amd/csrc/fcsa_kernels.h b/flash_cosine_sim_attention_amd/csrc/fcsa_kernels.h
--- a/flash_cosine_sim_attention_amd/csrc/fcsa_kernels.h
+++ b/flash_cosine_sim_attention_amd/csrc/fcsa_kernels.h
@@ -240,6 +240,8 @@
 int forward_wide128_mode(int set);
 hipError_t launch_forward_wide128(int dtype, const FwdParams& p, hipStream_t s);
 hipError_t launch_backward_dq(int dtype, int D, const BwdWinParams& p, hipStream_t s);
+int dq_rows64_mode(int set);
+hipError_t launch_backward_dq_rows64(int dtype, const BwdParams& p, hipStream_t s);
 hipError_t launch_backward_dbias(int dtype, int D, const BwdParams& p, hipStream_t s);
 hipError_t launch_backward_dkv(int dtype, int D, const BwdWinParams& p, hipStream_t s);
 int kv_group_mode(int set);
diff --git a/include/fcsa.h b/include/fcsa.h
--- a/include/fcsa.h
+++ b/include/fcsa.h
@@ -242,6 +242,8 @@
 
 int fcsa_debug_kv_group_form(int32_t form);
 
+int fcsa_debug_dq_form(int32_t form);
+
 const char* fcsa_last_error(void);
 
 #ifdef __cplusplus
```

New measurement: 767.5 (median of 6 runs). Within noise of the previous version (+0.4%).
